# ArthurBrussee/brush

Measured on AMD Instinct MI355X. Metric: train views/sec @ 1M Gaussians, 1080p (fwd + L1/SSIM loss + bwd + Adam per view), higher is better.
Workload: dtype f32

## Files before the change

brush_amd/_ffi.py:

```python
import ctypes as C
import os

_DIR = os.path.dirname(os.path.abspath(__file__))
LIB_PATH = os.environ.get("BRUSH_HIP_LIB") or os.path.join(_DIR, "libbrush_hip.so")

FLAG_MIP = 1
FLAG_BWD_INFO = 2
FLAG_SMOOTH_CUTOFF = 4
FLAG_SLICED_LISTS = 8

fp = C.POINTER(C.c_float)
u32p = C.POINTER(C.c_uint32)


class BhCamera(C.Structure):
    _fields_ = [
        ("vm", C.c_float * 12),
        ("fx", C.c_float), ("fy", C.c_float), ("cx", C.c_float), ("cy", C.c_float),
        ("lim_pos_x", C.c_float), ("lim_pos_y", C.c_float),
        ("lim_neg_x", C.c_float), ("lim_neg_y", C.c_float),
        ("cam_pos", C.c_float * 3),
        ("img_w", C.c_uint32), ("img_h", C.c_uint32),
        ("tile_row_begin", C.c_uint32), ("tile_row_end", C.c_uint32),
        ("model", C.c_uint32), ("dist", C.c_float * 8), ("half_max_render_fov", C.c_float),
# ... 372 lines not shown
    "bh_train_set_features": (C.c_int, [C.c_void_p, C.POINTER(BhFeatureField), C.POINTER(BhFeatureTarget)]),
    "bh_refine_carry_rows": (C.c_int, [C.c_void_p, C.c_void_p, C.c_void_p, C.c_uint32, C.c_uint32]),
}

REGION_BOX, REGION_ELLIPSOID = 0, 1


class BhSceneTransform(C.Structure):
    _fields_ = [("q", C.c_double * 4), ("t", C.c_double * 3), ("s", C.c_double), ("rot", C.c_float * 9), ("quat", C.c_float * 4),
                ("trans", C.c_float * 3), ("scale", C.c_float), ("log_scale", C.c_float), ("sh_rot", C.c_float * 164),
                ("reserved", C.c_uint32 * 2)]


class BhSceneRegion(C.Structure):
    _fields_ = [("kind", C.c_uint32), ("invert", C.c_uint32), ("center", C.c_float * 3), ("half_extent", C.c_float * 3),
                ("rot", C.c_float * 9), ("min_raw_opacity", C.c_float), ("reserved", C.c_uint32)]


SCENE_SYMBOLS = {
    "bh_scene_transform_make": (C.c_int, [dp, dp, C.c_double, C.POINTER(BhSceneTransform)]),
    "bh_scene_transform_compose": (C.c_int, [C.POINTER(BhSceneTransform), C.POINTER(BhSceneTransform), C.POINTER(BhSceneTransform)]),
    "bh_scene_transform_invert": (C.c_int, [C.POINTER(BhSceneTransform), C.POINTER(BhSceneTransform)]),
    "bh_camera_apply_scene_transform": (C.c_int, [C.POINTER(BhCamera), C.POINTER(BhSceneTransform), C.POINTER(BhCamera)]),
    "bh_splats_transform": (C.c_int, [C.c_void_p, C.POINTER(BhSceneTransform), C.c_uint32, C.c_uint32] + [C.c_void_p] * 6),
    "bh_splats_select_region": (C.c_int, [C.c_void_p, C.POINTER(BhSceneRegion), C.c_void_p, C.c_void_p, C.c_uint32, C.c_void_p, u32p]),
}

LIFT_MAX_LABELS, LIFT_UNASSIGNED, LIFT_ANY_LABEL = 256, 255, 0xFFFFFFFF
LIFT_VOTE_ONE = 16777216.0


class BhLiftSelect(C.Structure):
    _fields_ = [("label", C.c_uint32), ("min_share", C.c_float), ("min_weight", C.c_float), ("min_max_weight", C.c_float),
                ("min_pixels", C.c_uint32), ("invert", C.c_uint32)]


LIFT_SYMBOLS = {
    "bh_lift_accumulate": (C.c_int, [C.c_void_p, C.POINTER(BhRenderOut), C.c_void_p, C.c_uint32, C.c_void_p, C.c_void_p, C.c_void_p]),
    "bh_lift_assign": (C.c_int, [C.c_void_p, C.c_void_p, C.c_uint32, C.c_uint32, C.c_float, C.c_void_p, C.c_void_p]),
    "bh_lift_select": (C.c_int, [C.c_void_p, C.c_void_p, C.c_void_p, C.c_void_p, C.c_uint32, C.c_uint32, C.POINTER(BhLiftSelect), C.c_void_p]),
}

ENVMAP_MAX_RESOLUTION = 1024
ENVMAP_SYMBOLS = {
    "bh_envmap_create": (C.c_int, [C.c_void_p, C.c_uint32, C.POINTER(C.c_void_p)]),
    "bh_envmap_destroy": (C.c_int, [C.c_void_p, C.c_void_p]),
    "bh_envmap_set_params": (C.c_int, [C.c_void_p, C.c_void_p, fp]),
    "bh_envmap_get_params": (C.c_int, [C.c_void_p, C.c_void_p, fp]),
    "bh_envmap_get_grad": (C.c_int, [C.c_void_p, C.c_void_p, fp]),
    "bh_envmap_get_state": (C.c_int, [C.c_void_p, C.c_void_p, fp, fp, u32p]),
    "bh_envmap_set_state": (C.c_int, [C.c_void_p, C.c_void_p, fp, fp, C.c_uint32]),
    "bh_envmap_set_adam": (C.c_int, [C.c_void_p, C.c_void_p, C.c_double, C.c_double, C.c_double, C.c_double]),
    "bh_envmap_composite": (C.c_int, [C.c_void_p, C.c_void_p, C.POINTER(BhCamera), C.c_void_p, C.c_uint32, C.c_uint32, C.c_void_p]),
    "bh_envmap_backward": (C.c_int, [C.c_void_p, C.c_void_p, C.POINTER(BhCamera), C.c_void_p, C.c_void_p, C.c_uint32, C.c_uint32, C.c_void_p, C.c_int]),
    "bh_train_set_envmap": (C.c_int, [C.c_void_p, C.c_void_p]),
}

class BhCameraGradTerms(C.Structure):
    _fields_ = [("v_depth", C.c_void_p), ("v_normal", C.c_void_p), ("v_distortion", C.c_void_p), ("depth_mode", C.c_uint32),
                ("normal_mode", C.c_uint32), ("distortion", BhDistortionConfig)]


INTRINSICS_SYMBOLS = {
    "bh_render_backward_intrinsics_saved": (C.c_int, [C.c_void_p, C.POINTER(BhRenderOut)] + [C.c_void_p] * 10),
    "bh_render_backward_camera_saved": (C.c_int, [C.c_void_p, C.POINTER(BhRenderOut), C.c_void_p, C.POINTER(BhCameraGradTerms)] + [C.c_void_p] * 9),
    "bh_train_set_intrinsics_grad": (C.c_int, [C.c_void_p, C.c_void_p]),
    "bh_camera_set_intrinsics": (C.c_int, [C.POINTER(BhCamera), C.c_double, C.c_double, C.c_double, C.c_double]),
}

ABI_VERSION = 7
STRUCT_MIRRORS = (BhCamera, BhRenderOut, BhLossConfig, BhTrainConfig, BhTrainState, BhTrainBatch, BhTrainStats, BhRefineConfig, BhRefineStats, BhPlyInfo)

_lib = None
_lib_th = None
TEST_HOOKS_LIB_PATH = os.path.join(_DIR, "libbrush_hip_testhooks.so")
TEST_HOOK_SYMBOLS = {"bh_debug_fill_train_scratch": (C.c_int, [C.c_void_p, C.c_uint32]),
                     "bh_debug_split_counts": (C.c_int, [C.c_void_p, C.POINTER(C.c_uint32)]),
                     "bh_debug_depth_sort": (C.c_int, [C.c_void_p, C.c_void_p, C.c_void_p, C.c_void_p, C.c_uint32, C.c_void_p, C.c_void_p, C.c_void_p, C.c_void_p,
                                                       C.POINTER(C.c_int), C.POINTER(C.c_uint32)]),
                     "bh_debug_depth_deal": (C.c_int, [C.c_void_p, C.c_void_p, C.c_void_p, C.c_void_p, C.c_uint32, C.c_void_p, C.c_void_p, C.c_void_p, C.c_void_p,
                                                       C.c_uint32, C.c_uint32, C.POINTER(C.c_uint64), C.POINTER(C.c_int)]),
                     "bh_debug_dsort_deal_counts": (C.c_int, [C.c_void_p, C.POINTER(C.c_uint32)]),
                     "bh_debug_set_deal_capacity": (C.c_int, [C.c_void_p, C.c_uint32]),
                     "bh_debug_image_loss_window": (C.c_int, [C.c_void_p, C.c_void_p, C.c_void_p, C.c_uint32, C.c_uint32, C.POINTER(BhLossConfig), C.c_float, C.c_uint32,
                                                              C.c_uint32, C.c_void_p, C.c_void_p])}


class BrushHipError(RuntimeError):
    pass


def _bind(path, symbols):
    if not os.path.exists(path):
        raise BrushHipError(
            "%s not found: build it with `python -c 'import __graft_entry__ as g; g.build()'` "
            "(hipcc --offload-arch=gfx950). There is no CPU fallback." % path)
    lib = C.CDLL(path)
    for name, (res, args) in symbols.items():
        fn = getattr(lib, name)
        fn.restype = res
        fn.argtypes = args
    if lib.bh_abi_version() != ABI_VERSION:
        raise BrushHipError("%s speaks ABI %d, this binding ABI %d" % (path, lib.bh_abi_version(), ABI_VERSION))
    for i, mirror in enumerate(STRUCT_MIRRORS):
        if lib.bh_struct_size(i) != C.sizeof(mirror):
            raise BrushHipError("%s: sizeof(%s) is %d in the library, %d in this binding" % (path, mirror.__name__, lib.bh_struct_size(i), C.sizeof(mirror)))
    return lib


def load():
    global _lib
    if _lib is None:
        _lib = _bind(LIB_PATH, dict(SYMBOLS, **LPIPS_SYMBOLS, **COMPRESSED_PLY_SYMBOLS, **IMAGE_SYMBOLS, **DEPTH_SYMBOLS, **POSE_SYMBOLS, **EXPOSURE_SYMBOLS, **BILAGRID_SYMBOLS, **DEPTH_LOSS_SYMBOLS, **NORMAL_SYMBOLS, **NORMAL_LOSS_SYMBOLS, **DISTORTION_SYMBOLS, **MESH_SYMBOLS, **SPARSE_MESH_SYMBOLS, **FEATURE_SYMBOLS, **FEATURE_TRAIN_SYMBOLS, **SCENE_SYMBOLS, **LIFT_SYMBOLS, **ENVMAP_SYMBOLS, **INTRINSICS_SYMBOLS))
    return _lib


def load_test_hooks():
    global _lib_th
    if _lib_th is None:
        _lib_th = _bind(TEST_HOOKS_LIB_PATH, dict(SYMBOLS, **LPIPS_SYMBOLS, **COMPRESSED_PLY_SYMBOLS, **IMAGE_SYMBOLS, **DEPTH_SYMBOLS, **POSE_SYMBOLS, **EXPOSURE_SYMBOLS, **BILAGRID_SYMBOLS, **DEPTH_LOSS_SYMBOLS, **NORMAL_SYMBOLS, **NORMAL_LOSS_SYMBOLS, **DISTORTION_SYMBOLS, **MESH_SYMBOLS, **SPARSE_MESH_SYMBOLS, **FEATURE_SYMBOLS, **FEATURE_TRAIN_SYMBOLS, **SCENE_SYMBOLS, **LIFT_SYMBOLS, **ENVMAP_SYMBOLS, **INTRINSICS_SYMBOLS,
                                                   **TEST_HOOK_SYMBOLS))
    return _lib_th
```

brush_amd/csrc/api.hip:

```cpp
#include <cmath>
#include <cstdlib>
#include <cstdio>
#include <algorithm>
#include <cstring>
#include <new>

#include "../../include/brush_hip_intrinsics.h"
#include "context.h"
#include "depth_deal.h"
#include "device_rng.h"
#include "param_table.h"

namespace bh {

__global__ __launch_bounds__(256) void zero_two_kernel(float4* __restrict__ a, size_t na, float4* __restrict__ b, size_t nb) {
    const size_t stride = (size_t)gridDim.x * 256;
    const float4 z = make_float4(0.0f, 0.0f, 0.0f, 0.0f);
    for (size_t i = (size_t)blockIdx.x * 256 + threadIdx.x; i < na + nb; i += stride) {
        if (i < na) a[i] = z;
        else b[i - na] = z;
    }
}

int set_error(bh_ctx* ctx, int code, const std::string& msg) {
// ... 166 lines not shown

uint32_t bh_struct_size(uint32_t which) {
    switch (which) {
        case BH_STRUCT_CAMERA: return (uint32_t)sizeof(BhCamera);
        case BH_STRUCT_RENDER_OUT: return (uint32_t)sizeof(BhRenderOut);
        case BH_STRUCT_LOSS_CONFIG: return (uint32_t)sizeof(BhLossConfig);
        case BH_STRUCT_TRAIN_CONFIG: return (uint32_t)sizeof(BhTrainConfig);
        case BH_STRUCT_TRAIN_STATE: return (uint32_t)sizeof(BhTrainState);
        case BH_STRUCT_TRAIN_BATCH: return (uint32_t)sizeof(BhTrainBatch);
        case BH_STRUCT_TRAIN_STATS: return (uint32_t)sizeof(BhTrainStats);
        case BH_STRUCT_REFINE_CONFIG: return (uint32_t)sizeof(BhRefineConfig);
        case BH_STRUCT_REFINE_STATS: return (uint32_t)sizeof(BhRefineStats);
        case BH_STRUCT_PLY_INFO: return (uint32_t)sizeof(BhPlyInfo);
        default: return 0u;
    }
}

bh_ctx* bh_create(int device, void* stream, int own_stream) {
    bh_ctx* ctx = new (std::nothrow) bh_ctx();
    if (!ctx) return nullptr;
    ctx->device = device;
    if (hipSetDevice(device) != hipSuccess) {
        (void)hipGetLastError();
        delete ctx;
        return nullptr;
    }
    if (!own_stream) {
        ctx->stream = (hipStream_t)stream;
        ctx->owns_stream = false;
    } else {
        if (hipStreamCreateWithFlags(&ctx->stream, hipStreamNonBlocking) != hipSuccess) {
            (void)hipGetLastError();
            delete ctx;
            return nullptr;
        }
        ctx->owns_stream = true;
    }
    if (hipHostMalloc((void**)&ctx->host_counters, bh::HOST_COUNTERS_BYTES, hipHostMallocCoherent)    != hipSuccess) {
        (void)hipGetLastError();
        if (ctx->owns_stream) (void)hipStreamDestroy(ctx->stream);
        delete ctx;
        return nullptr;
    }
    std::memset(ctx->host_counters, 0, bh::HOST_COUNTERS_BYTES);
#ifdef BH_TEST_HOOKS
    ctx->knob_break_allreduce = getenv("BH_BREAK_ALLREDUCE") != nullptr;
    if (ctx->knob_break_allreduce)
        fprintf(stderr, "brush_hip: BH_BREAK_ALLREDUCE is set - every all-reduce of this context's communicator is deliberately CORRUPTED (test hook)\n");
    if (const char* e = getenv("BH_TEST_FAIL_LOSS_AT")) {
        ctx->knob_fail_loss_at = (uint32_t)atoi(e);
        if (ctx->knob_fail_loss_at) fprintf(stderr, "brush_hip: BH_TEST_FAIL_LOSS_AT=%u - that train step of this context will FAIL on purpose (test hook)\n", ctx->knob_fail_loss_at);
    }
#endif
    if (hipEventCreateWithFlags(&ctx->readback_ev, hipEventDisableTiming) != hipSuccess ||
        hipEventCreateWithFlags(&ctx->gate_ev, hipEventDisableTiming) != hipSuccess) {
        if (ctx->readback_ev) (void)hipEventDestroy(ctx->readback_ev);
        (void)hipGetLastError();
        (void)hipHostFree(ctx->host_counters);
        if (ctx->owns_stream) (void)hipStreamDestroy(ctx->stream);
        delete ctx;
        return nullptr;
    }
    return ctx;
}

void bh_destroy(bh_ctx* ctx) {
    if (!ctx) return;
    (void)hipSetDevice(ctx->device);
    (void)hipStreamSynchronize(ctx->stream);
    prof_resolve(ctx);
    for (hipEvent_t e : ctx->prof.pool) (void)hipEventDestroy(e);
    for (auto& b : ctx->slots)
        if (b.ptr) (void)hipFree(b.ptr);
    for (auto& kv : ctx->views)
        if (kv.second.zcut) (void)hipFree(kv.second.zcut);
    for (auto& rt : ctx->retained)
        for (auto& b : rt.blocks)
            if (b.ptr) (void)hipFree(b.ptr);
    for (auto& b : ctx->pool)
        if (b.ptr) (void)hipFree(b.ptr);
    if (ctx->host_counters) (void)hipHostFree(ctx->host_counters);
    if (ctx->dsort_spl) (void)hipFree(ctx->dsort_spl);
    if (ctx->deal_ctr) (void)hipFree(ctx->deal_ctr);
    if (ctx->sort_groups) (void)hipFree(ctx->sort_groups);
    if (ctx->readback_ev) (void)hipEventDestroy(ctx->readback_ev);
    if (ctx->gate_ev) (void)hipEventDestroy(ctx->gate_ev);
    if (ctx->image_tab_host) (void)hipHostFree(ctx->image_tab_host);
    if (ctx->image_tab_ev) (void)hipEventDestroy(ctx->image_tab_ev);
    bh::param_tables_free_all(ctx);
    if (ctx->comm) (void)bh_comm_destroy(ctx);
    if (ctx->owns_stream) (void)hipStreamDestroy(ctx->stream);
    delete ctx;
}

const char* bh_last_error(bh_ctx* ctx) { return ctx ? ctx->last_error.c_str() : "null context"; }

int bh_sync(bh_ctx* ctx) {
    if (!ctx) return BH_ERR_INVALID_ARG;
    if (ctx->far_job.pending) {
        BH_HIP(ctx, hipSetDevice(ctx->device));
        BH_TRY(finish_far_slice(ctx, nullptr));
    }
    BH_HIP(ctx, hipStreamSynchronize(ctx->stream));
    deliver_pending_loss(ctx);
    return 0;
}

int bh_profile_enable(bh_ctx* ctx, int on) {
    if (!ctx) return BH_ERR_INVALID_ARG;
    ctx->prof.level = on < 0 ? 0 : (on > 2 ? 1 : on);
    return 0;
}

int bh_profile_fetch(bh_ctx* ctx, const char** names, float* ms, uint32_t* calls, int cap) {
    if (!ctx) return BH_ERR_INVALID_ARG;
    prof_resolve(ctx);
    Profiler& p = ctx->prof;
    const int n = p.count < cap ? p.count : cap;
    for (int i = 0; i < n; ++i) {
        names[i] = p.names[i];
        ms[i] = p.ms[i];
        calls[i] = p.calls[i];
    }
    p.count = 0;
    return n;
}

namespace {
bool parse_u32(const char* v, uint32_t lo, uint32_t hi, uint32_t* out) {
    if (!v || !*v) return false;
    char* end = nullptr;
    const unsigned long long x = strtoull(v, &end, 10);
    if (*end != '\0' || x < lo || x > hi) return false;
    *out = (uint32_t)x;
    return true;
}
bool parse_flag(const char* v, bool* out) {
    uint32_t x = 0;
    if (!parse_u32(v, 0, 1, &x)) return false;
    *out = x != 0;
    return true;
}
struct Option { const char* name; const char* help; bool (*apply)(bh_ctx* c, const char* v); };
const Option kOptions[] = {
    {"cut_min_pairs", "u32: a view whose last frame had fewer pairs keeps complete lists (= bh_set_list_cut_threshold)",
     [](bh_ctx* c, const char* v) { return parse_u32(v, 0, 0xFFFFFFFFu, &c->cut_min_pairs); }},
    {"cut_margin_pct", "0..10000: base margin behind a tile's last useful splat, % of its depth rank (default 150)",
     [](bh_ctx* c, const char* v) { return parse_u32(v, 0, 10000, &c->knob_cut_margin_pct); }},
    {"cut_margin_fixed", "0|1: the margin is cut_margin_pct for every frame instead of adaptive",
     [](bh_ctx* c, const char* v) { return parse_flag(v, &c->knob_fixed_margin); }},
    {"cut_ctrl", "up:down:floor:gap_exp — the margin controller's constants (default 1.5:0.998:0.5:0.3333)", [](bh_ctx* c, const char* v) {
        float a = 0, b = 0, d = 0, e = 0;
        if (sscanf(v, "%f:%f:%f:%f", &a, &b, &d, &e) != 4 || !(a >= 1.0f && b > 0.0f && b <= 1.0f && d > 0.0f && e >= 0.0f && e <= 1.0f)) return false;
        c->ctrl_up = a; c->ctrl_down = b; c->ctrl_floor = d; c->ctrl_gap_exp = e;
        return true;
    }},
    {"cut_sort_all", "0|1: with per-tile cuts, still depth-sort every visible splat",
     [](bh_ctx* c, const char* v) { return parse_flag(v, &c->knob_cut_sort_all); }},
    {"auto_exact_share", "0..1: a view whose last cut frame listed more than this share of its pairs renders complete lists (default 0.9; 0 = never)", [](bh_ctx* c, const char* v) {
        char* end = nullptr;
        const float x = strtof(v, &end);
        if (end == v || *end != '\0' || !(x >= 0.0f && x <= 1.0f)) return false;
        c->auto_exact_share = x;
        return true;
    }},
    {"no_view_hash", "0|1: frames without a view id share ONE table instead of being keyed by their camera",
     [](bh_ctx* c, const char* v) { return parse_flag(v, &c->knob_no_view_hash); }},
    {"k16_order", "0 index order | 1 by the view's last per-tile work | 2 dealt: the forward blend's tile order",
     [](bh_ctx* c, const char* v) { return parse_u32(v, 0, 2, &c->knob_k16_order); }},
    {"band_mode", "0|1: XCD bands of the blend kernels — contiguous eighths of the tile range, or dealt in chunks of 8 adjacent tiles (default 1)",
     [](bh_ctx* c, const char* v) { return parse_u32(v, 0, 1, &c->knob_band_mode); }},
    {"k16_waves", "0..8: forward blend: resident one-wave tiles per SIMD (0 = 8 = all resident at once; fewer: the lighter tiles are dispatched as the heavier ones finish)",
     [](bh_ctx* c, const char* v) { return parse_u32(v, 0, 8, &c->knob_k16_waves); }},
    {"k16_split", "0..1000: forward blend: a tile whose forecast work is at least max(256, k16_split / 100 x its band's mean) is blended by four quadrant waves (default 250; 0: no tile is split)",
     [](bh_ctx* c, const char* v) { return parse_u32(v, 0, 1000, &c->knob_k16_split); }},
    {"k16_split_of_max", "0..100: ... and at least this many percent of its band's heaviest tile (default 45)",
     [](bh_ctx* c, const char* v) { return parse_u32(v, 0, 100, &c->knob_k16_split_of_max); }},
    {"k16_split_min", "1..1023: a tile below this many blended splats (forecast) is never split (default 256)",
     [](bh_ctx* c, const char* v) { return parse_u32(v, 1, 1023, &c->knob_k16_split_min); }},
    {"k5_exact_spw", "16|32|64: splats per wave of the list builder for complete lists",
     [](bh_ctx* c, const char* v) { uint32_t u = 0; if (!parse_u32(v, 16, 64, &u) || !(u == 16 || u == 32 || u == 64)) return false; c->knob_k5_exact_spw = u; return true; }},
    {"bwd_jobs", "0|1: the blend backward works on checkpointed 128-entry segments of the tiles' lists (default 1) or on whole tiles",
     [](bh_ctx* c, const char* v) { return parse_flag(v, &c->knob_bwd_jobs); }},
    {"bwd_wide_rows", "0|1: the blend backward addresses the gradient accumulator in 64 bits, as it does by itself from 2^32 bytes of accumulator on (default 0)",
     [](bh_ctx* c, const char* v) { return parse_flag(v, &c->knob_bwd_wide_rows); }},
    {"no_lpt", "0|1: the blend backward takes its tiles in index order",
     [](bh_ctx* c, const char* v) { return parse_flag(v, &c->knob_no_lpt); }},
    {"lpt_classes", "log|linear: work classes of the backward's longest-first tile order — two per octave of blended splats, or 1/64 of the mean list length wide",
     [](bh_ctx* c, const char* v) { const std::string w(v); if (w == "log") { c->knob_lpt_linear = false; return true; } if (w == "linear") { c->knob_lpt_linear = true; return true; } return false; }},
    {"generic_depth_sort", "0|1: depth order by the generic radix sort + scan instead of the fused split sort",
     [](bh_ctx* c, const char* v) { return parse_flag(v, &c->knob_generic_depth_sort); }},
    {"dsort_splitters", "0|1: the fused depth sort splits at the 254 depth quantiles of the view's previous frame (default 1) or always linearly over the frame's key range",
     [](bh_ctx* c, const char* v) { return parse_flag(v, &c->knob_dsort_splitters); }},
    {"dsort_deal", "0|1: K1 deals the listed splats straight into the depth sort's buckets when the view's splitter table holds quantiles (default 1) or the histogram and split launches always run",
     [](bh_ctx* c, const char* v) { return parse_flag(v, &c->knob_dsort_deal); }},
    {"tile_sort", "auto|bucket|lsd: the forward's tile sort (auto: bucket sort unless the view's pairs are concentrated in few tiles)",
     [](bh_ctx* c, const char* v) { const std::string w(v); if (w == "auto") { c->knob_tile_sort = 0; return true; } if (w == "bucket") { c->knob_tile_sort = 1; return true; } if (w == "lsd") { c->knob_tile_sort = 2; return true; } return false; }},
    {"spec_k5", "0|1: queue the list builder before the host has read the frame's counts (default 1; 0: behind the count readback)",
     [](bh_ctx* c, const char* v) { return parse_flag(v, &c->knob_spec_k5); }},
    {"event_waits", "0|1: the host's mid-step waits use events behind the kernels instead of polled tag words",
     [](bh_ctx* c, const char* v) { return parse_flag(v, &c->knob_event_waits); }},
    {"readback_copy", "0|1: counts and gate word reach the host through copy launches",
     [](bh_ctx* c, const char* v) { return parse_flag(v, &c->knob_readback_copy); }},
    {"force_exchange", "0|1: a one-rank communicator still walks the whole gradient-exchange path (overhead measurement)",
     [](bh_ctx* c, const char* v) { return parse_flag(v, &c->knob_force_exchange); }},
    {"zero_grads", "0|1: the single-GPU train step zero-fills its gradient span like the exchange path",
     [](bh_ctx* c, const char* v) { return parse_flag(v, &c->knob_zero_grads); }},
    {"loss_bands", "0|1: the fused loss's blocks take their tiles by XCD column bands (1) or row-major (0)",
     [](bh_ctx* c, const char* v) { return parse_u32(v, 0, 1, &c->knob_loss_bands); }},
    {"update_rows", "0|64|128|256: splats per block of the update kernel (0 = default)",
     [](bh_ctx* c, const char* v) { uint32_t u = 0; if (!parse_u32(v, 0, 256, &u) || !(u == 0 || u == 64 || u == 128 || u == 256)) return false; c->knob_update_rows = u; return true; }},
    {"no_dormant", "0|1: the update kernel fetches and updates dormant splats like everyone else",
     [](bh_ctx* c, const char* v) { return parse_flag(v, &c->knob_no_dormant); }},
    {"sort_kpt", "0|4|8|16: keys per thread of the generic radix sort (0 = default)",
     [](bh_ctx* c, const char* v) { uint32_t u = 0; if (!parse_u32(v, 0, 16, &u) || !(u == 0 || u == 4 || u == 8 || u == 16)) return false; c->knob_sort_kpt = u; return true; }},
    {"grad_allreduce", "ring|direct: the dense gradient block's collective — ncclAllReduce, or reduce-scatter + all-gather over grouped send/recv",
     [](bh_ctx* c, const char* v) { const std::string w(v); if (w == "ring") { c->knob_direct_allreduce = false; return true; } if (w == "direct") { c->knob_direct_allreduce = true; return true; } return false; }},
    {"update_sparse", "0..256: an update block with at most this many non-dormant rows fetches them in one round trip (0: never; 256: every block that may skip dormant rows; default 64 at SH degree 0, else 0)",
     [](bh_ctx* c, const char* v) { uint32_t u = 0; if (!parse_u32(v, 0, 256, &u)) return false; c->knob_update_sparse = (int)u; return true; }},
    {"feature_chunk", "0|4|8|16: channels per pass over the lists of the feature-map blends (0 = chosen per channel count)",
     [](bh_ctx* c, const char* v) { uint32_t u = 0; if (!parse_u32(v, 0, 16, &u) || !(u == 0 || u == 4 || u == 8 || u == 16)) return false; c->feature_chunk = u; return true; }},
};
constexpr int kOptionCount = (int)(sizeof(kOptions) / sizeof(kOptions[0]));
}

extern "C" int bh_option_count(void) { return kOptionCount; }
extern "C" const char* bh_option_name(int i) { return i >= 0 && i < kOptionCount ? kOptions[i].name : nullptr; }
extern "C" const char* bh_option_help(int i) { return i >= 0 && i < kOptionCount ? kOptions[i].help : nullptr; }

extern "C" int bh_set_option(bh_ctx* ctx, const char* key, const char* value) {
    if (!ctx) return BH_ERR_INVALID_ARG;
    if (!key || !value) return set_error(ctx, BH_ERR_INVALID_ARG, "set_option: null key or value");
    const std::string k(key);
    for (const Option& o : kOptions) {
        if (k != o.name) continue;
        if (!o.apply(ctx, value)) return set_error(ctx, BH_ERR_INVALID_ARG, "set_option: bad value '" + std::string(value) + "' for '" + k + "'");
        return 0;
    }
    return set_error(ctx, BH_ERR_INVALID_ARG, "set_option: unknown key '" + k + "' (bh_option_name lists the keys)");
}

namespace {
struct Kb4Law {
    double k[4];
    explicit Kb4Law(const float* d) { for (int i = 0; i < 4; ++i) k[i] = d ? (double)d[i] : 0.0; }
    double value(double th) const {
        const double t2 = th * th, t3 = t2 * th, t5 = t3 * t2, t7 = t5 * t2, t9 = t7 * t2;
        return th + k[0] * t3 + k[1] * t5 + k[2] * t7 + k[3] * t9;
    }
    double slope(double th) const {
        const double t2 = th * th, t4 = t2 * t2, t6 = t4 * t2, t8 = t6 * t2;
        return 1.0 + 3.0 * k[0] * t2 + 5.0 * k[1] * t4 + 7.0 * k[2] * t6 + 9.0 * k[3] * t8;
    }
    double invert(double target) const {
        if (target <= 0.0) return 0.0;
        const double pi = 3.14159265358979323846;
        double th = target < pi - 1e-6 ? target : pi - 1e-6;
        for (int it = 0; it < 50; ++it) {
            const double fp = slope(th);
            if (std::fabs(fp) < 1e-12) break;
            double next = th - (value(th) - target) / fp;
            next = next < 0.0 ? 0.0 : (next > pi ? pi : next);
            const bool done = std::fabs(next - th) < 1e-12;
            th = next;
            if (done) break;
        }
        return th;
    }
};
struct Rt8Law {
    double k[6];
    explicit Rt8Law(const float* d) { for (int i = 0; i < 6; ++i) k[i] = d ? (double)d[i] : 0.0; }
    double radial(double r) const {
        const double r2 = r * r, r4 = r2 * r2, r6 = r4 * r2;
        return (1.0 + k[0] * r2 + k[1] * r4 + k[2] * r6) / (1.0 + k[3] * r2 + k[4] * r4 + k[5] * r6);
    }
    double undistort(double r_d) const {
        double r = r_d;
// ... 136 lines not shown

extern "C" int bh_render_forward(bh_ctx* ctx, const BhCamera* cam, uint32_t n, uint32_t sh_degree, const float* transforms,
                                 const float* sh_coeffs, const float* raw_opacities, const float* background, uint32_t flags,
                                 BhRenderOut* out) {
    if (!ctx) return BH_ERR_INVALID_ARG;
    if (!cam || !out || !background) return set_error(ctx, BH_ERR_INVALID_ARG, "render_forward: null argument");
    ForwardRequest req;
    req.cam = *cam;
    req.n = n; req.sh_degree = sh_degree; req.flags = flags;
    req.transforms = transforms; req.sh_coeffs = sh_coeffs; req.raw_opacities = raw_opacities;
    req.bg[0] = background[0]; req.bg[1] = background[1]; req.bg[2] = background[2];
    req.view_id = ctx->view_id;
    return render_forward(ctx, req, out);
}

int bh::forward_impl(bh_ctx* ctx, const ForwardRequest& req, BhRenderOut* out) {
    const uint32_t n = req.n, sh_degree = req.sh_degree, flags = req.flags;
    const float* transforms = req.transforms;
    const float* sh_coeffs = req.sh_coeffs;
    const float* raw_opacities = req.raw_opacities;
    ctx->have_forward = false;
    ctx->clears.begin_forward();
    const bool mip = flags & BH_FLAG_MIP;
    Frame f;
    f.bwd_info = flags & BH_FLAG_BWD_INFO; f.smooth = flags & BH_FLAG_SMOOTH_CUTOFF;
    f.bg[0] = req.bg[0]; f.bg[1] = req.bg[1]; f.bg[2] = req.bg[2];
    f.u = make_uniforms(req.cam);
    if (f.u.tile_y0 >= f.u.tile_y1 || f.u.tile_y1 > f.u.tile_bh) return set_error(ctx, BH_ERR_INVALID_ARG, "tile_row window must satisfy begin < end <= ceil(img_h / 16)");
    f.num_tiles = f.u.tile_bw * f.u.tile_bh;
    const size_t npad = n ? n : 1;

    constexpr size_t counter_set_bytes = COUNTER_SET_BYTES, counter_set_words = COUNTER_SET_BYTES / 4, counter_read_bytes = COUNTER_READ_BYTES;
    auto* counter_pairs = (uint32_t*)ensure(ctx, SLOT_COUNTERS, 2 * counter_set_bytes + 64);
    uint32_t* dev_sums = counter_pairs ? counter_pairs + 2 * counter_set_words : nullptr;
    uint32_t* counters = counter_pairs ? counter_pairs + counter_set_words * (ctx->counter_phase & 1u) : nullptr;
    auto* depth_keys = (uint32_t*)ensure(ctx, SLOT_DEPTH_KEYS, npad * 4);
    auto* isect_counts = (uint32_t*)ensure(ctx, SLOT_ISECT_COUNTS, npad * 4);
    auto* max_radius = req.max_radius ? req.max_radius : (float*)ensure(ctx, SLOT_MAX_RADIUS, npad * 4);
    f.proj_by_gid = (float*)ensure(ctx, SLOT_PROJECTED_BY_GID, npad * 9 * 4);
    if (!counters || !depth_keys || !isect_counts || !max_radius || !f.proj_by_gid) return BH_ERR_OOM;

    f.gfc = (uint32_t*)ensure(ctx, SLOT_GLOBAL_FROM_COMPACT, npad * 4);
    auto* depths_sorted = (uint32_t*)ensure(ctx, SLOT_DEPTHS_SORTED, npad * 4);
    if (!f.gfc || !depths_sorted) return BH_ERR_OOM;
    const bool bwd_jobs = f.bwd_info && ctx->knob_bwd_jobs && !ctx->knob_no_lpt && !((flags & BH_FLAG_SLICED_LISTS) && ctx->slice_fraction > 0.0f);
    const size_t lpt_words = LPT_HEADER_WORDS + (size_t)8 * LPT_CLASSES * band_slots(f.num_tiles);
    auto* tile_offsets = (uint32_t*)ensure(ctx, SLOT_TILE_OFFSETS, ((size_t)f.num_tiles * 2 + lpt_words) * 4);
    f.visible = (f.bwd_info && req.visible) ? req.visible : (float*)ensure(ctx, SLOT_VISIBLE, (f.bwd_info ? npad : 1) * 4);
    if (!tile_offsets || !f.visible) return BH_ERR_OOM;
    const size_t visible_words = f.bwd_info ? ((req.visible && req.visible_floats) ? req.visible_floats : npad) : 0;
    const bool want_sliced = (flags & BH_FLAG_SLICED_LISTS) != 0;
    const size_t slice_bit_words = ((size_t)f.num_tiles + 31) / 32;
    const size_t slice_group_words = (size_t)n / (256 * FAR_GROUP_BLOCKS) + 2;
    const size_t slice_words = want_sliced ? SLICE_CTRL_WORDS + slice_bit_words + (size_t)f.num_tiles * 2 + slice_group_words : 0;
    uint32_t* slice_tab = nullptr;
    if (want_sliced) {
        slice_tab = (uint32_t*)ensure(ctx, SLOT_SLICE, slice_words * 4);
        if (!slice_tab) return BH_ERR_OOM;
    }
    ViewState* view = nullptr;
    bool cut_active = false;
    const bool auto_cuts = want_sliced && !(ctx->slice_fraction > 0.0f);
    const bool order_only = !want_sliced && ctx->knob_k16_order != 0u && n >= 8u * 256u;
    if (n > 0 && (auto_cuts || order_only)) {
        view = frame_view(ctx, req, f.u.tile_bw, f.u.tile_bh, order_only && !f.bwd_info);
        if (!view && auto_cuts) return set_error(ctx, BH_ERR_OOM, "hipMalloc for the per-view tile table failed");
        if (!view) (void)hipGetLastError();
        cut_active = auto_cuts && view && cut_this_frame(ctx, view, req.allow_cut);
    }
    uint32_t* const vtab = view_table(view);
    uint32_t* near_counts = nullptr;
    uint32_t* tile_order = nullptr;
    uint32_t* tile_split = nullptr;
    if (cut_active) {
        near_counts = (uint32_t*)ensure(ctx, SLOT_NEAR_COUNTS, npad * 4);
        if (!near_counts) return BH_ERR_OOM;
    }

    uint32_t near_total = 0, nv_true = 0;
    bool fused_scan = false;
    uint32_t* cum_early = nullptr;
    bool k5_queued = false;
    uint32_t spec_pair_cap = 0;
    float* spec_projected = nullptr;
    float4* spec_vc = nullptr;
    uint32_t *spec_tile_ids = nullptr, *spec_isect_gids = nullptr;
    if (n > 0) {
        fused_scan = depth_sort_supported(n) && !ctx->knob_generic_depth_sort;
        const bool sums_on_device = fused_scan && !ctx->knob_readback_copy;
        bool* spl_written = nullptr;
        uint32_t* spl_listed = nullptr;
        uint32_t* spl = view_splitters(view, cut_active, &spl_written, &spl_listed);
        if (!spl && ctx->dsort_spl) { spl = ctx->dsort_spl; spl_written = &ctx->dsort_spl_written; spl_listed = &ctx->dsort_spl_keys; }
        DealArgs dealt;
        {
            ProfScope ps(ctx, "ProjectSplats");
            if (!ctx->counters_ready) BH_HIP(ctx, hipMemsetAsync(counter_pairs, 0, 2 * counter_set_bytes, ctx->stream));
            ctx->counters_ready = false;
            ForwardPrep prep;
            prep.next_counters = reinterpret_cast<unsigned long long*>(counter_pairs + counter_set_words * ((ctx->counter_phase & 1u) ^ 1u));
            prep.visible = visible_words ? reinterpret_cast<uint32_t*>(f.visible) : nullptr;
            prep.visible_words = (uint32_t)visible_words;
            prep.tile_table = tile_offsets;
            prep.tile_words = f.num_tiles * 2 + LPT_HEADER_WORDS;
            prep.slice_table = slice_tab;
            prep.slice_words = (uint32_t)slice_words;
            prep.list_all_visible = ctx->knob_cut_sort_all;
            if (view && ctx->knob_k16_order && n >= 8u * 256u) {
                const uint32_t win_t = f.u.tile_bw * (f.u.tile_y1 - f.u.tile_y0);
                tile_order = (uint32_t*)ensure(ctx, SLOT_TILE_ORDER, ((size_t)8 * band_slots(win_t) + SPLIT_TAIL_WORDS) * 4);
                if (!tile_order) return BH_ERR_OOM;
                prep.order_work = vtab + (size_t)f.num_tiles;
                prep.order_out = tile_order;
                prep.order_tiles = win_t;
                prep.order_tile_begin = f.u.tile_bw * f.u.tile_y0;
                prep.order_mode = ctx->knob_k16_order;
                prep.band_mode = ctx->knob_band_mode;
                if (ctx->knob_k16_split && ctx->knob_k16_order == 1u) {
                    tile_split = tile_order + (size_t)8 * band_slots(win_t);
                    prep.split_out = tile_split;
                    prep.split_factor = (float)ctx->knob_k16_split * 0.01f;
                    prep.split_min = ctx->knob_k16_split_min;
                    prep.split_of_max = (float)ctx->knob_k16_split_of_max * 0.01f;
                }
            }
            if (f.bwd_info && req.grad_begin && req.grad_floats && (req.grad_floats & 3u) == 0 &&
                (reinterpret_cast<uintptr_t>(req.grad_begin) & 15u) == 0 && req.grad_floats / 4 <= 0xFFFFFFFFull) {
                prep.span = reinterpret_cast<float4*>(req.grad_begin);
                prep.span_f4 = (uint32_t)(req.grad_floats / 4);
                ctx->clears.k1_cleared_span();
            }
            BH_TRY(depth_deal_prepare(ctx, n, spl, sums_on_device && spl_written && *spl_written && depth_deal_table_usable(*spl_listed), &prep));
            dealt = prep.deal;
            BH_TRY(launch_project_forward(ctx, f.u, n, mip, sh_degree, transforms, sh_coeffs, raw_opacities, depth_keys, isect_counts, max_radius,
                                          f.proj_by_gid, counters, prep, cut_active ? vtab : nullptr, near_counts));
            ctx->counter_phase ^= 1u;
            ctx->counters_ready = true;
        }
        auto* hslots = reinterpret_cast<unsigned long long*>(ctx->host_counters + 16);
        const bool poll_tag = sums_on_device && !ctx->knob_event_waits;
        if (!sums_on_device) {
            BH_HIP(ctx, hipMemcpyAsync(hslots, counters, counter_read_bytes, hipMemcpyDeviceToHost, ctx->stream));
            BH_HIP(ctx, hipEventRecord(ctx->readback_ev, ctx->stream));
        }
        {
            ProfScope ps(ctx, "DepthSort");
            if (fused_scan) {
                cum_early = (uint32_t*)ensure(ctx, SLOT_CUM_TILES_HIT, npad * 4);
                if (!cum_early) return BH_ERR_OOM;
                if (poll_tag && ++ctx->readback_tag == 0u) ctx->readback_tag = 1u;
                BH_TRY(depth_sort_scan(ctx, depth_keys, counters + COUNTER_MINMAX_WORD, cut_active ? near_counts : isect_counts, n, depths_sorted, f.gfc, cum_early,
                                       sums_on_device ? counters : nullptr, ctx->host_counters + 16, ctx->readback_ev, poll_tag ? ctx->readback_tag : 0u,
                                       sums_on_device ? dev_sums : nullptr, spl, spl_written, &dealt));
            } else {
                BH_TRY(radix_argsort(ctx, depth_keys, nullptr, n, 32, depths_sorted, f.gfc));
            }
        }
        if (poll_tag && ctx->knob_spec_k5 && !(want_sliced && ctx->slice_fraction > 0.0f)) {
            const size_t cap_pairs = std::min(ctx->slots[SLOT_TILE_IDS].cap, ctx->slots[SLOT_ISECT_GIDS].cap) / 4;
            if (cap_pairs >= 4096) {
                spec_projected = (float*)ensure(ctx, SLOT_PROJECTED, npad * 9 * 4);
                spec_vc = f.bwd_info ? (float4*)ensure(ctx, SLOT_V_COMBINED, npad * 10 * 4 + 16) : nullptr;
                if (!spec_projected || (f.bwd_info && !spec_vc)) return BH_ERR_OOM;
                spec_tile_ids = (uint32_t*)ctx->slots[SLOT_TILE_IDS].ptr;
                spec_isect_gids = (uint32_t*)ctx->slots[SLOT_ISECT_GIDS].ptr;
                spec_pair_cap = (uint32_t)std::min<size_t>(cap_pairs, 0xFFFFFFFEull);
                ProfScope ps(ctx, "MapGaussiansToIntersect");
                BH_TRY(launch_map_gaussians(ctx, n, f.u, f.proj_by_gid, f.gfc, spec_projected, cum_early, spec_tile_ids, spec_isect_gids, spec_vc,
                                            spec_vc ? (uint32_t)(((size_t)n * 10 + 3) / 4) : 0u, 0xFFFFFFFFu, cut_active ? slice_tab : nullptr,
                                            cut_active ? vtab : nullptr, cut_active ? depths_sorted : nullptr, dev_sums + (cut_active ? 3 : 0), spec_pair_cap));
                k5_queued = true;
            }
        }
        if (poll_tag) BH_TRY(wait_host_tag(ctx, reinterpret_cast<const volatile uint32_t*>(hslots) + HOST_SUM_WORDS - 1u, ctx->readback_tag, "count readback"));
        else BH_HIP(ctx, hipEventSynchronize(ctx->readback_ev));
        if (ctx->gate_learn) {
            ctx->gate_learn = false;
            ctx->far_direct = reinterpret_cast<const volatile uint32_t*>(ctx->host_counters)[HOST_GATE_WORD] != 0u;
        }
        unsigned long long hc[4] = {0ull, 0ull, 0ull, 0ull};
        if (sums_on_device) {
            const volatile unsigned long long* hs = hslots;
            for (uint32_t c = 0; c < COUNTER_K1_U64; ++c) hc[c] = hs[c];
        } else {
            for (uint32_t k = 0; k < COUNTER_SLOTS; ++k)
                for (uint32_t c = 0; c < COUNTER_K1_U64; ++c) hc[c] += hslots[COUNTER_K1_U64 * k + c];
        }
        if (hc[1] > 0xFFFFFFFFull) return set_error(ctx, BH_ERR_UNSUPPORTED, "more than 2^32-1 tile intersections");
        nv_true = (uint32_t)hc[0];
        f.ni = (uint32_t)hc[1];
        near_total = cut_active ? (uint32_t)hc[2] : f.ni;
        f.nv = cut_active ? (uint32_t)hc[3] : nv_true;
        if (dealt.ctr && reinterpret_cast<const volatile uint32_t*>(hslots)[HOST_DEAL_WORD] != 0u) {
            ProfScope ps(ctx, "DepthSort");
            ctx->deal_fallbacks++;
            BH_TRY(depth_sort_scan(ctx, depth_keys, counters + COUNTER_MINMAX_WORD, cut_active ? near_counts : isect_counts, n, depths_sorted, f.gfc, cum_early,
                                   counters, ctx->host_counters + 16, ctx->readback_ev, 0u, dev_sums, spl, spl_written));
            k5_queued = false;
        }
        if (fused_scan && spl_listed && (spl_written == nullptr || *spl_written)) *spl_listed = f.nv;
    } else {
        BH_HIP(ctx, hipMemsetAsync(tile_offsets, 0, ((size_t)f.num_tiles * 2 + LPT_HEADER_WORDS) * 4, ctx->stream));
        if (visible_words) BH_HIP(ctx, hipMemsetAsync(f.visible, 0, visible_words * 4, ctx->stream));
    }

    const size_t nvpad = f.nv ? f.nv : 1, nipad = f.ni ? f.ni : 1;
    f.cum = fused_scan ? cum_early : (uint32_t*)ensure(ctx, SLOT_CUM_TILES_HIT, nvpad * 4);
    f.projected = (float*)ensure(ctx, SLOT_PROJECTED, nvpad * 9 * 4);
    f.tile_ids = (uint32_t*)ensure(ctx, SLOT_TILE_IDS, nipad * 4);
    f.isect_gids = (uint32_t*)ensure(ctx, SLOT_ISECT_GIDS, nipad * 4);
    f.tile_ids_sorted = (uint32_t*)ensure(ctx, SLOT_TILE_IDS_SORTED, nipad * 4);
    f.isect_gids_sorted = (uint32_t*)ensure(ctx, SLOT_ISECT_GIDS_SORTED, nipad * 4);
    const size_t pixels = (size_t)f.u.img_w * f.u.img_h;
    void* out_img = ensure(ctx, SLOT_OUT_IMG, pixels * (f.bwd_info ? 16 : 4));
    if (!f.cum || !f.projected || !f.tile_ids || !f.isect_gids || !f.tile_ids_sorted || !f.isect_gids_sorted || !out_img)
        return BH_ERR_OOM;
    if (k5_queued && ((cut_active ? near_total : f.ni) > spec_pair_cap || f.projected != spec_projected || f.tile_ids != spec_tile_ids || f.isect_gids != spec_isect_gids))
        k5_queued = false;

    f.budget = want_sliced && f.ni > 0 ? list_budget(ctx, cut_active ? view : nullptr, near_total, f.ni) : f.ni;
    const bool sliced = f.budget < f.ni;
    const bool by_cut = cut_active && sliced;
    const uint32_t* zcut_lists = cut_active ? vtab : nullptr;
    f.slice_info = slice_tab;
    f.done_bits = slice_tab ? slice_tab + SLICE_CTRL_WORDS : nullptr;
    f.tile_offsets_far = slice_tab ? slice_tab + SLICE_CTRL_WORDS + slice_bit_words : nullptr;
    f.far_group_totals = slice_tab ? slice_tab + SLICE_CTRL_WORDS + slice_bit_words + (size_t)f.num_tiles * 2 : nullptr;
    while (f.tile_bits < 32 && (f.num_tiles >> f.tile_bits) != 0) f.tile_bits++;
    if (bwd_jobs) {
        const uint32_t listed = cut_active ? near_total : f.ni;
        const uint32_t ckpt_cap = (uint32_t)std::min<uint64_t>((uint64_t)listed / BWD_SEG + f.num_tiles + 1u, BWD_CKPT_MAX_SLOTS);
        f.rs.jobs.ckpt = (float4*)ensure(ctx, SLOT_BWD_CKPT, (size_t)ckpt_cap * 256 * sizeof(float4));
        f.rs.jobs.ckpt_cap = ckpt_cap;
        f.rs.jobs.top_cap = band_slots(f.num_tiles) + ckpt_cap;
        f.rs.jobs.top_list = (uint32_t*)ensure(ctx, SLOT_BWD_TOPLIST, (size_t)8 * f.rs.jobs.top_cap * 4);
        if (!f.rs.jobs.ckpt || !f.rs.jobs.top_list) return BH_ERR_OOM;
    }
    if (view) {
        f.rs.zcut = vtab;
        f.rs.depth_keys_sorted = depths_sorted;
        f.rs.nv = f.nv;
        f.rs.cut_active = by_cut;
        f.rs.margin_pct = cut_margin_pct(ctx, view);
        f.rs.work = vtab + (size_t)f.num_tiles;
        f.rs.order = tile_order;
        f.rs.order_mode = ctx->knob_k16_order;
        f.rs.split = tile_split;
#ifdef BH_TEST_HOOKS
        ctx->last_split = tile_split;
#endif
    }
    const uint32_t win_tiles = f.u.tile_bw * (f.u.tile_y1 - f.u.tile_y0);
    const float class_width_raw = (float)f.ni / (float)(win_tiles ? win_tiles : 1u) / 64.0f;
    f.class_width = ctx->knob_lpt_linear ? (class_width_raw < 8.0f ? 8.0f : class_width_raw) : 0.0f;
    f.lpt = (f.bwd_info && !ctx->knob_no_lpt) ? tile_offsets + (size_t)f.num_tiles * 2 : nullptr;
    f.out_f32 = f.bwd_info ? (float*)out_img : nullptr;
    f.out_u8 = f.bwd_info ? nullptr : (uint32_t*)out_img;

    bool offsets_done = false;
    if (f.nv > 0) {
        if (!fused_scan) {
            ProfScope ps(ctx, "PrefixSumGaussHits");
            BH_TRY(prefix_sum(ctx, cut_active ? near_counts : isect_counts, f.gfc, f.nv, f.cum, false));
        }
        if (f.ni == 0) {
            ProfScope ps(ctx, "ProjectVisible");
            BH_TRY(launch_project_visible(ctx, f.nv, f.proj_by_gid, f.gfc, f.projected));
        }
        if (f.ni > 0) {
            {
                ProfScope ps(ctx, "MapGaussiansToIntersect");
                float4* vc = nullptr;
                if (f.bwd_info) {
                    vc = (float4*)ensure(ctx, SLOT_V_COMBINED, (size_t)f.nv * 10 * 4 + 16);
                    if (!vc) return BH_ERR_OOM;
                }
                if (zcut_lists && near_total == 0u) {
                } else if (k5_queued && (!f.bwd_info || vc == spec_vc)) {
                    ctx->clears.k5_cleared_accum(vc != nullptr);
                } else {
                    ctx->clears.k5_cleared_accum(vc != nullptr);
                    BH_TRY(launch_map_gaussians(ctx, f.nv, f.u, f.proj_by_gid, f.gfc, f.projected, f.cum, f.tile_ids, f.isect_gids, vc, vc ? (uint32_t)(((size_t)f.nv * 10 + 3) / 4) : 0u,
                                                (sliced && !by_cut) ? f.budget : 0xFFFFFFFFu, (sliced || zcut_lists) ? f.slice_info : nullptr, zcut_lists,
                                                zcut_lists ? depths_sorted : nullptr));
                }
            }
            {
                ProfScope ps(ctx, "TileSort");
                if ((zcut_lists || !sliced) && tile_sort_supported(f.tile_bits, zcut_lists ? near_total : f.ni) && !(ctx->knob_tile_sort == 2u)) {
                    BH_TRY(tile_sort_offsets(ctx, f.tile_ids, f.isect_gids, zcut_lists ? near_total : f.ni, f.tile_bits, f.num_tiles, f.tile_ids_sorted, f.isect_gids_sorted,
                                             tile_offsets, f.ni));
                    offsets_done = true;
                } else
                if (zcut_lists) BH_TRY(radix_argsort_dev(ctx, f.tile_ids, f.isect_gids, near_total, nullptr, nullptr, nullptr, f.tile_bits, f.tile_ids_sorted, f.isect_gids_sorted, f.ni));
                else if (sliced) BH_TRY(radix_argsort_dev(ctx, f.tile_ids, f.isect_gids, f.budget, f.slice_info + 1, nullptr, nullptr, f.tile_bits, f.tile_ids_sorted, f.isect_gids_sorted, f.ni));
                else BH_TRY(radix_argsort(ctx, f.tile_ids, f.isect_gids, f.ni, f.tile_bits, f.tile_ids_sorted, f.isect_gids_sorted));
            }
        }
    }
    if (!offsets_done) {
        ProfScope ps(ctx, "GetTileOffsets");
        if (zcut_lists) BH_TRY(launch_tile_offsets(ctx, f.tile_ids_sorted, near_total, f.num_tiles, tile_offsets, true));
        else if (sliced) BH_TRY(launch_tile_offsets_dev(ctx, f.tile_ids_sorted, f.budget, f.slice_info + 1, nullptr, nullptr, f.num_tiles, tile_offsets));
        else BH_TRY(launch_tile_offsets(ctx, f.tile_ids_sorted, f.ni, f.num_tiles, tile_offsets, true));
    }
    if (!sliced) {
        ProfScope ps(ctx, "Rasterize");
        BH_TRY(launch_rasterize(ctx, f.u, f.bg, f.bwd_info, f.smooth, f.isect_gids_sorted, tile_offsets, f.projected, f.gfc, f.out_f32, f.out_u8, f.visible, f.lpt,
                                f.class_width, 0, &f.rs));
    } else {
        auto* state = (float*)ensure(ctx, SLOT_SLICE_STATE, pixels * 16);
        f.far_counts = (uint32_t*)ensure(ctx, SLOT_SLICE_COUNTS, nvpad * 4);
        f.far_block_totals = (uint32_t*)ensure(ctx, SLOT_SLICE_CUM, (nvpad / 256 + 2) * 4);
        if (!state || !f.far_counts || !f.far_block_totals) return BH_ERR_OOM;
        f.rs.done_bits = f.done_bits;
        f.rs.unsat_count = f.slice_info + 2;
        if (!ctx->knob_readback_copy) {
            f.rs.gate_host = ctx->host_counters + HOST_GATE_WORD;
            *reinterpret_cast<volatile uint32_t*>(f.rs.gate_host) = 0u;
        }
        f.rs.state = state;
        f.rs.offsets_near = tile_offsets;
        f.rs.live_bands = f.slice_info + 4;
        {
            ProfScope ps(ctx, "Rasterize");
            BH_TRY(launch_rasterize(ctx, f.u, f.bg, f.bwd_info, f.smooth, f.isect_gids_sorted, tile_offsets, f.projected, f.gfc, f.out_f32, f.out_u8, f.visible, f.lpt,
                                    f.class_width, 1, &f.rs));
        }
        FarJob& j = ctx->far_job;
        j.frame = f;
        j.by_cut = by_cut;
        j.view = by_cut ? view : nullptr;
        j.view_shared = req.view_id == 0u && ctx->knob_no_view_hash;
        if (by_cut) j.req = req;
        if (ctx->knob_readback_copy)
            BH_HIP(ctx, hipMemcpyAsync(ctx->host_counters + HOST_GATE_WORD, f.slice_info + 2, 4, hipMemcpyDeviceToHost, ctx->stream));
        if (ctx->far_direct && !by_cut) {
            BH_TRY(enqueue_far_slice(ctx, j));
            ctx->gate_learn = true;
        } else {
            if (++ctx->gate_tag == 0u) ctx->gate_tag = 1u;
            j.gate_tag = ctx->gate_tag;
            ctx->gate_signal_queued = false;
            j.gate_event_recorded = !(req.defer_decision && !ctx->knob_event_waits && !ctx->knob_readback_copy);
            if (j.gate_event_recorded) BH_HIP(ctx, hipEventRecord(ctx->gate_ev, ctx->stream));
            j.pending = true;
            if (!req.defer_decision) {
                bool again = false;
                BH_TRY(finish_far_slice(ctx, &again));
                if (by_cut && again) {
                    *out = ctx->latest.out;
                    return 0;
                }
            }
        }
    }

    BhRenderOut r{};
    r.num_visible = nv_true;
    r.num_listed_splats = f.nv;
    r.num_intersections = f.ni;
    r.num_tiles = f.num_tiles;
    r.tile_bw = f.u.tile_bw;
    r.tile_bh = f.u.tile_bh;
// ... 403 lines not shown
    if (n == 0) return 0;
    if (tile_sort_supported(bits, n) && !(ctx->knob_tile_sort == 2u))
        return tile_sort_offsets(ctx, tile_ids, compact_gids, n, bits, num_tiles, tile_ids_sorted, compact_gids_sorted, tile_offsets);
    BH_TRY(radix_argsort(ctx, tile_ids, compact_gids, n, bits, tile_ids_sorted, compact_gids_sorted));
    return launch_tile_offsets(ctx, tile_ids_sorted, n, num_tiles, tile_offsets, true);
}

#ifdef BH_TEST_HOOKS
extern "C" int bh_debug_split_counts(bh_ctx* ctx, uint32_t* out) {
    if (!ctx || !out) return BH_ERR_INVALID_ARG;
    if (!ctx->last_split) return 0;
    BH_HIP(ctx, hipSetDevice(ctx->device));
    BH_HIP(ctx, hipMemcpyAsync(out, ctx->last_split, 8 * 4, hipMemcpyDeviceToHost, ctx->stream));
    BH_HIP(ctx, hipStreamSynchronize(ctx->stream));
    return 1;
}
extern "C" int bh_debug_depth_sort(bh_ctx* ctx, const uint32_t* keys, const uint32_t* minmax, const uint32_t* counts, uint32_t n, uint32_t* out_keys, uint32_t* out_vals,
                                   uint32_t* cum, uint32_t* spl, int* spl_written, uint32_t* totals_out) {
    if (!ctx) return BH_ERR_INVALID_ARG;
    if (!keys || !minmax || !counts || !out_keys || !out_vals || !cum || !totals_out || (spl && !spl_written))
        return set_error(ctx, BH_ERR_INVALID_ARG, "debug_depth_sort: null argument");
    if (n == 0 || !depth_sort_supported(n)) return set_error(ctx, BH_ERR_INVALID_ARG, "debug_depth_sort: n is outside the fused sort's reach");
    BH_HIP(ctx, hipSetDevice(ctx->device));
    bool written = spl_written ? *spl_written != 0 : false;
    BH_TRY(depth_sort_scan(ctx, keys, minmax, counts, n, out_keys, out_vals, cum, nullptr, nullptr, nullptr, 0u, nullptr, spl, spl ? &written : nullptr));
    if (spl) *spl_written = written ? 1 : 0;
    else if (spl_written) *spl_written = ctx->dsort_spl_written ? 1 : 0;
    BH_HIP(ctx, hipMemcpyAsync(totals_out, ctx->slots[SLOT_SORT_HIST].ptr, 2 * 256 * 4, hipMemcpyDeviceToHost, ctx->stream));
    BH_HIP(ctx, hipStreamSynchronize(ctx->stream));
    return 0;
}
__global__ __launch_bounds__(256) void debug_deal_kernel(const uint32_t* __restrict__ keys, const uint32_t* __restrict__ counts, uint32_t n, uint32_t stride, bh::DealArgs d) {
    __shared__ uint32_t s_spl[bh::DEAL_SPL_WORDS];
    bh::deal_stage(d, s_spl);
    __syncthreads();
    const uint32_t t = blockIdx.x * 256u + threadIdx.x;
    if (t >= n) return;
    const uint32_t e = (uint32_t)(((unsigned long long)t * stride) % n);
    const uint32_t key = keys[e];
    if (key != 0xFFFFFFFFu) bh::deal_put(d, bh::deal_take(d, s_spl, key, counts[e]), key, e);
}
extern "C" int bh_debug_depth_deal(bh_ctx* ctx, const uint32_t* keys, const uint32_t* minmax, const uint32_t* counts, uint32_t n, uint32_t* out_keys, uint32_t* out_vals,
                                   uint32_t* cum, uint32_t* spl, uint32_t cap, uint32_t stride, unsigned long long* ctr_out, int* fell_back) {
    if (!ctx) return BH_ERR_INVALID_ARG;
    if (!keys || !minmax || !counts || !out_keys || !out_vals || !cum || !spl || !ctr_out || !fell_back || stride == 0u)
        return set_error(ctx, BH_ERR_INVALID_ARG, "debug_depth_deal: bad argument");
    if (n == 0 || !depth_sort_supported(n)) return set_error(ctx, BH_ERR_INVALID_ARG, "debug_depth_deal: n is outside the fused sort's reach");
    BH_HIP(ctx, hipSetDevice(ctx->device));
    DealArgs d;
    d.spl = spl;
    d.cap = cap ? cap : deal_capacity(n);
    d.region = (uint2*)ensure(ctx, SLOT_DEAL_REGION, (size_t)DEAL_BUCKETS * d.cap * sizeof(uint2));
    if (!d.region) return BH_ERR_OOM;
    if (hipMalloc((void**)&d.ctr, (size_t)DEAL_SET_U64 * 8) != hipSuccess) { (void)hipGetLastError(); return BH_ERR_OOM; }
    int rc = check_hip(ctx, hipMemsetAsync(d.ctr, 0, (size_t)DEAL_SET_U64 * 8, ctx->stream), "debug_depth_deal: clear");
    if (rc == 0) {
        hipLaunchKernelGGL(debug_deal_kernel, dim3((n + 255u) / 256u), dim3(256), 0, ctx->stream, keys, counts, n, stride, d);
        rc = check_hip(ctx, hipGetLastError(), "debug_deal_kernel");
    }
    bool written = true;
    if (rc == 0) rc = depth_sort_scan(ctx, keys, minmax, counts, n, out_keys, out_vals, cum, nullptr, nullptr, nullptr, 0u, nullptr, spl, &written, &d);
    unsigned long long host[DEAL_BUCKETS + 1u];
    if (rc == 0) rc = check_hip(ctx, hipMemcpy2DAsync(host, 8, d.ctr, (size_t)DEAL_LINE_U64 * 8, 8, DEAL_BUCKETS + 1u, hipMemcpyDeviceToHost, ctx->stream), "debug_depth_deal: counters");
    if (rc == 0) rc = check_hip(ctx, hipStreamSynchronize(ctx->stream), "debug_depth_deal: sync");
    if (rc == 0) {
        for (uint32_t i = 0; i <= DEAL_BUCKETS; ++i) ctr_out[i] = host[i];
        *fell_back = host[DEAL_BUCKETS] != 0ull ? 1 : 0;
        if (*fell_back) {
            ctx->deal_fallbacks++;
            rc = depth_sort_scan(ctx, keys, minmax, counts, n, out_keys, out_vals, cum, nullptr, nullptr, nullptr, 0u, nullptr, spl, &written);
            if (rc == 0) rc = check_hip(ctx, hipStreamSynchronize(ctx->stream), "debug_depth_deal: sync");
        }
    } else {
        (void)hipStreamSynchronize(ctx->stream);
    }
    (void)hipFree(d.ctr);
    return rc;
}
extern "C" int bh_debug_set_deal_capacity(bh_ctx* ctx, uint32_t cap) {
    if (!ctx) return BH_ERR_INVALID_ARG;
    ctx->deal_cap_override = cap;
    return 0;
}
extern "C" int bh_debug_dsort_deal_counts(bh_ctx* ctx, uint32_t* out) {
    if (!ctx || !out) return BH_ERR_INVALID_ARG;
    out[0] = ctx->deal_frames;
    out[1] = ctx->deal_fallbacks;
    return 0;
}
extern "C" int bh_debug_image_loss_window(bh_ctx* ctx, const float* img_hwc4, const uint32_t* gt_packed, uint32_t h, uint32_t w, const BhLossConfig* cfg,
                                          float alpha_weight, uint32_t tile_y0, uint32_t tile_y1, float* loss_out, float* v_output) {
    if (!ctx) return BH_ERR_INVALID_ARG;
    if (!img_hwc4 || !gt_packed || !cfg || !loss_out || !v_output || h == 0 || w == 0)
        return set_error(ctx, BH_ERR_INVALID_ARG, "debug_image_loss_window: bad argument");
    if (tile_y0 >= tile_y1) return set_error(ctx, BH_ERR_INVALID_ARG, "debug_image_loss_window: empty tile-row window");
    BH_HIP(ctx, hipSetDevice(ctx->device));
    const size_t hw = (size_t)h * w;
    const bool alpha = alpha_weight > 0.0f;
    BH_TRY(launch_image_loss_fused_window(ctx, img_hwc4, gt_packed, h, w, *cfg, alpha, 1.0f / (float)(hw * 3), alpha ? alpha_weight / (float)hw : 0.0f, tile_y0,
                                          tile_y1, loss_out, v_output, nullptr, nullptr, 0u));
    BH_HIP(ctx, hipStreamSynchronize(ctx->stream));
    return 0;
}
#endif
```

brush_amd/csrc/context.h:

```cpp
#pragma once
#include <hip/hip_runtime.h>
#include <stdint.h>

#include <memory>
#include <string>
#include <unordered_map>
#include <vector>

#include "../../include/brush_hip.h"
#include "../../include/brush_hip_lpips.h"
#include "../../include/brush_hip_image.h"
#include "../../include/brush_hip_exposure.h"
#include "../../include/brush_hip_bilagrid.h"
#include "../../include/brush_hip_depth_loss.h"
#include "../../include/brush_hip_normal_loss.h"
#include "../../include/brush_hip_distortion.h"
#include "../../include/brush_hip_mesh.h"
#include "../../include/brush_hip_features.h"
#include "../../include/brush_hip_feature_train.h"
#include "../../include/brush_hip_envmap.h"
#include "device_math.h"

namespace bh {

enum Slot : int {
    SLOT_COUNTERS = 0,
    SLOT_DEPTH_KEYS,
    SLOT_ISECT_COUNTS,
    SLOT_MAX_RADIUS,
    SLOT_SORT_KEYS_A,
    SLOT_SORT_KEYS_B,
    SLOT_SORT_VALS_A,
    SLOT_SORT_VALS_B,
    SLOT_SORT_HIST,
    SLOT_COMM_SCRATCH,
    SLOT_BWD_CKPT,
    SLOT_BWD_TOPLIST,
    SLOT_SORT_PARTS,
    SLOT_SCAN_SUMS,
    SLOT_GLOBAL_FROM_COMPACT,
    SLOT_DEPTHS_SORTED,
    SLOT_CUM_TILES_HIT,
    SLOT_PROJECTED,
    SLOT_TILE_IDS,
    SLOT_ISECT_GIDS,
    SLOT_TILE_IDS_SORTED,
    SLOT_ISECT_GIDS_SORTED,
    SLOT_TILE_OFFSETS,
    SLOT_OUT_IMG,
    SLOT_VISIBLE,
    SLOT_V_COMBINED,
    SLOT_LOSS_MAP,
    SLOT_V_OUTPUT,
    SLOT_GRADS,
    SLOT_STATS,
    SLOT_LOSS_SCALAR,
    SLOT_MISC,
    SLOT_REFINE,
    SLOT_REFINE_BOUNDS,
    SLOT_FOLDED_TRANSFORMS,
    SLOT_FOLDED_RAW_OPAC,
    SLOT_PLY_ROWS,
    SLOT_EXCH_BLOCKS,
    SLOT_EXCH_IDX,
    SLOT_EXCH_COMPACT,
    SLOT_PROJECTED_BY_GID,
    SLOT_SLICE,
    SLOT_SLICE_STATE,
    SLOT_SLICE_COUNTS,
    SLOT_SLICE_CUM,
    SLOT_NEAR_COUNTS,
    SLOT_TILE_ORDER,
    SLOT_LOD_GRADS,
    SLOT_LOD_FOLDED,
    SLOT_LOD_LOSS,
    SLOT_LOD_SORT,
    SLOT_KNN,
    SLOT_EVAL,
    SLOT_LPIPS,
    SLOT_PLY_COMPRESS,
    SLOT_IMAGE,
    SLOT_DEPTH,
    SLOT_POSE,
    SLOT_INTRINSICS,
    SLOT_EXPOSURE,
    SLOT_CORRECTED,
    SLOT_PIXEL_LOSS,
    SLOT_DEPTH_TERM,
    SLOT_NORMAL,
    SLOT_NORMAL_TERM,
    SLOT_DISTORTION,
    SLOT_DISTORTION_TERM,
    SLOT_BILAGRID,
    SLOT_TSDF,
    SLOT_FEATURES,
    SLOT_FEATURE_TERM,
    SLOT_FEATURE_GRAD,
    SLOT_ENVMAP_FRAME,
    SLOT_DEAL_REGION,
    SLOT_SCENE,
    SLOT_SPTSDF,
    SLOT_COUNT
};

struct Buffer {
    void* ptr = nullptr;
    size_t cap = 0;
};

constexpr int MAX_PROF = 32;

constexpr uint32_t COUNTER_SLOTS = 128;
constexpr uint32_t COUNTER_K1_U64 = 4;
constexpr size_t COUNTER_SET_BYTES = COUNTER_SLOTS * 8 * COUNTER_K1_U64 + COUNTER_SLOTS * 8;
constexpr uint32_t COUNTER_SET_U64 = (uint32_t)(COUNTER_SET_BYTES / 8);
constexpr uint32_t COUNTER_MINMAX_WORD = COUNTER_SLOTS * 2 * COUNTER_K1_U64;
constexpr uint32_t SLICE_CTRL_WORDS = 8;
constexpr uint32_t SORT_GROUP_BLOCKS = 32;
constexpr uint32_t FAR_GROUP_BLOCKS = 64;
constexpr size_t COUNTER_READ_BYTES = COUNTER_SLOTS * 8 * COUNTER_K1_U64;
constexpr uint32_t HOST_SUM_WORDS = 2 * COUNTER_K1_U64 + 1;
constexpr uint32_t HOST_DEAL_WORD = HOST_SUM_WORDS;
constexpr size_t HOST_LOSS_WORD = 16 + COUNTER_READ_BYTES / 4;
constexpr size_t HOST_GATE_WORD = HOST_LOSS_WORD + 16;
constexpr size_t HOST_GATE_TAG_WORD = HOST_GATE_WORD + 1;
constexpr size_t HOST_COUNTERS_BYTES = 64 + COUNTER_READ_BYTES + 64 + 64;

struct Profiler {
    int level = 0;
    const char* names[MAX_PROF];
    float ms[MAX_PROF];
    uint32_t calls[MAX_PROF];
    int count = 0;
    struct Pending { int idx; hipEvent_t a, b; };
    std::vector<Pending> pending;
    std::vector<hipEvent_t> pool;
    hipEvent_t ext_a = nullptr, ext_b = nullptr;
};

constexpr uint32_t ZCUT_ALL = 0xFFFFFFFEu;
BH_DEV bool zcut_near(uint32_t key, uint32_t cut) { return (key >> 1) <= (cut >> 1); }
struct ViewState {
    uint32_t* zcut = nullptr;
    uint32_t tile_bw = 0, tile_bh = 0;
    bool seeded = false;
    uint32_t exact_frames = 0;
    uint32_t penalty = 0;
    uint64_t last_used = 0;
    uint32_t gap = 0;
    uint32_t last_pairs = 0;
    uint32_t complete_frames = 0;
    bool spl_written[2] = {false, false};
    uint32_t spl_keys[2] = {0, 0};
    bool casual = false;
};
constexpr uint32_t CUT_MIN_PAIRS = 1500000u;
constexpr uint32_t LPT_CLASSES = 64;
constexpr uint32_t LPT_HEADER_WORDS = 8 * LPT_CLASSES + 64;
constexpr uint32_t BWD_SEG = 128;
constexpr uint32_t BWD_MAX_SEGS = 64;
struct BwdJobs {
    float4* ckpt = nullptr;
    uint32_t ckpt_cap = 0;
    uint32_t* top_list = nullptr;
    uint32_t top_cap = 0;
};
constexpr uint32_t BAND_CHUNK = 4;
inline __host__ __device__ uint32_t band_slots(uint32_t num_tiles) {
    const uint32_t p = (num_tiles + 7u) / 8u;
    return ((p + BAND_CHUNK - 1u) / BAND_CHUNK) * BAND_CHUNK;
}
inline __host__ __device__ uint32_t band_tile(uint32_t band, uint32_t i, uint32_t per, uint32_t mode) {
    return mode ? ((i / BAND_CHUNK) * 8u + band) * BAND_CHUNK + (i % BAND_CHUNK) : band * per + i;
}
BH_DEV uint32_t tile_of_block(uint32_t b, uint32_t num_tiles, uint32_t band_mode) {
    const uint32_t per = band_slots(num_tiles);
    const uint32_t i = b >> 3;
    return i < per ? band_tile(b & 7u, i, per, band_mode) : 0xFFFFFFFFu;
}
constexpr uint32_t SPLIT_MAX = 128;
constexpr uint32_t SPLIT_MIN_WORK = 256;
constexpr uint32_t SPLIT_TAIL_WORDS = 8u + 8u * SPLIT_MAX * 4u;
constexpr uint32_t BWD_CKPT_MAX_SLOTS = 96u * 1024u;
constexpr uint32_t DSORT_SPL_STRIDE = 260;
constexpr uint32_t VIEW_SPL_WORDS = 2 * DSORT_SPL_STRIDE;
constexpr uint32_t DEAL_BUCKETS = 255;
constexpr uint32_t DEAL_LINE_U64 = 16;
constexpr uint32_t DEAL_SET_U64 = (DEAL_BUCKETS + 1u) * DEAL_LINE_U64;
constexpr uint32_t DEAL_OVERFLOW_U64 = DEAL_BUCKETS * DEAL_LINE_U64;
struct DealArgs {
    const uint32_t* spl = nullptr;
    unsigned long long* ctr = nullptr;
    uint2* region = nullptr;
    uint32_t cap = 0;
};
constexpr size_t MAX_VIEW_STATES = 4096;
constexpr uint64_t DIRECT_ALLREDUCE_MIN_FLOATS = 1u << 16;
constexpr uint32_t AUTO_EXACT_FRAMES = 12;
constexpr size_t CASUAL_VIEW_STATES = 32;
constexpr size_t SEEN_KEYS = 64;
constexpr size_t VIEW_TABLE_BYTES = (size_t)256 << 20;

struct RasterSlice {
    uint32_t* done_bits = nullptr;
    uint32_t* unsat_count = nullptr;
    uint32_t* gate_host = nullptr;
    float* state = nullptr;
    const uint32_t* offsets_near = nullptr;
    uint32_t* zcut = nullptr;
    const uint32_t* depth_keys_sorted = nullptr;
    uint32_t nv = 0;
    bool cut_active = false;
    uint32_t* live_bands = nullptr;
    uint32_t* work = nullptr;
    const uint32_t* order = nullptr;
    uint32_t order_mode = 1;
    uint32_t* split = nullptr;
    uint32_t margin_pct = 150;
    BwdJobs jobs{};
};

struct ForwardRequest {
    BhCamera cam{};
    uint32_t n = 0, sh_degree = 0, flags = 0;
    const float* transforms = nullptr;
    const float* sh_coeffs = nullptr;
    const float* raw_opacities = nullptr;
    float bg[3] = {0, 0, 0};
    uint32_t view_id = 0;
    float* visible = nullptr;
    float* max_radius = nullptr;
    size_t visible_floats = 0;
    float* grad_begin = nullptr;
    size_t grad_floats = 0;
    bool defer_decision = false;
    bool allow_cut = true;
};

struct Frame {
    ViewUniforms u{};
    float bg[3] = {0, 0, 0};
    bool bwd_info = false, smooth = false;
    uint32_t nv = 0, ni = 0, budget = 0, num_tiles = 0, tile_bits = 0;
    float* proj_by_gid = nullptr;
    uint32_t* gfc = nullptr;
    float* projected = nullptr;
    uint32_t* cum = nullptr;
    uint32_t* slice_info = nullptr;
    uint32_t* done_bits = nullptr;
    uint32_t* tile_offsets_far = nullptr;
    uint32_t* far_counts = nullptr;
    uint32_t* far_block_totals = nullptr;
    uint32_t* far_group_totals = nullptr;
    uint32_t* tile_ids = nullptr;
    uint32_t* isect_gids = nullptr;
    uint32_t* tile_ids_sorted = nullptr;
    uint32_t* isect_gids_sorted = nullptr;
    float* out_f32 = nullptr;
    uint32_t* out_u8 = nullptr;
    float* visible = nullptr;
    uint32_t* lpt = nullptr;
    float class_width = 8.0f;
    RasterSlice rs{};
};

struct FarJob {
    bool pending = false;
    Frame frame{};
    bool gate_event_recorded = false;
    uint32_t gate_tag = 0;
    bool by_cut = false;
    ViewState* view = nullptr;
    bool view_shared = false;
    ForwardRequest req{};
};

struct GradClears {
// ... 78 lines not shown
    float* pose_grad = nullptr;
    float* intrinsics_grad = nullptr;
    bool depth_attached = false;
    BhDepthTarget depth_target{};
    bool normal_attached = false;
    BhNormalTermConfig normal_term{};
    bool distortion_attached = false;
    BhDistortionTermConfig distortion_term{};
    bool feature_attached = false;
    BhFeatureField feature_field{};
    BhFeatureTarget feature_target{};
    bh_exposure* exposure = nullptr;
    bh_bilagrid* bilagrid = nullptr;
    float bilagrid_tv_weight = 0.0f;
    bh_envmap* envmap = nullptr;

    bool lpips_on() const { return lpips != nullptr && lpips_weight > 0.0f; }
    bool depth_on() const { return depth_attached && depth_target.weight > 0.0f; }
    bool normal_on() const { return normal_attached && normal_term.weight > 0.0f; }
    bool distortion_on() const { return distortion_attached; }
    bool feature_on() const { return feature_attached && feature_target.weight > 0.0f; }
};

}


struct bh_ctx {
    int device = 0;
    hipStream_t stream = nullptr;
    bool owns_stream = false;
    std::string last_error;
    bh::Buffer slots[bh::SLOT_COUNT];
    uint32_t* host_counters = nullptr;
    hipEvent_t readback_ev = nullptr;
    hipEvent_t gate_ev = nullptr;
    bool counters_ready = false;
    uint32_t counter_phase = 0;
    bool have_forward = false;
    bh::ForwardState latest;
    uint64_t generation = 0;
    std::vector<bh::Retained> retained;
    std::vector<bh::Buffer> pool;
    bh::GradClears clears;
    float* pending_loss_dst = nullptr;
    void* image_tab_host = nullptr;
    size_t image_tab_cap = 0;
    hipEvent_t image_tab_ev = nullptr;
    bh::StepTerms terms;
    std::vector<bh::ParamTable*> param_tables;
    void* comm = nullptr;
    hipStream_t comm_stream = nullptr;
    hipEvent_t comm_ev = nullptr;
    int comm_rank = 0, comm_world = 1;
    float slice_fraction = 0.0f;
    float last_slice_share = 1.0f;
    bool far_direct = false;
    uint32_t readback_tag = 0;
    uint32_t gate_tag = 0;
    bool gate_signal_queued = false;
    bool gate_learn = false;
    uint32_t far_launches = 0;
    std::unordered_map<uint64_t, bh::ViewState> views;
    uint64_t seen_keys[bh::SEEN_KEYS] = {};
    uint32_t seen_pos = 0;
    uint32_t casual_views = 0;
    uint32_t view_id = 0;
    uint64_t view_clock = 0;
    float margin_scale = 1.0f;
    float ctrl_up = 1.5f, ctrl_down = 0.998f, ctrl_floor = 0.5f, ctrl_gap_exp = 1.0f / 3.0f;
    uint32_t cut_min_pairs = bh::CUT_MIN_PAIRS;
    bool knob_spec_k5 = true;
    bool knob_event_waits = false;
    bool knob_readback_copy = false;
    bool knob_no_view_hash = false;
    bool knob_fixed_margin = false;
    bool knob_cut_sort_all = false;
    uint32_t feature_chunk = 0;
    uint32_t knob_band_mode = 1;
    uint32_t knob_k16_waves = 0;
    uint32_t knob_k16_split = 250;
    uint32_t knob_k16_split_min = bh::SPLIT_MIN_WORK;
    uint32_t knob_k16_split_of_max = 45;
    const uint32_t* last_split = nullptr;
    uint32_t knob_k16_order = 1;
    uint32_t knob_cut_margin_pct = 150;
    bh::FarJob far_job;
    uint32_t refine_n = 0, refine_new_n = 0;
    bool dsort_deal_lds_raised = false;
    bool dsort_lds_raised = false;
    uint32_t* sort_groups = nullptr;
    size_t sort_groups_cap = 0, sort_groups_dirty = 0;
    uint32_t sort_groups_cur = 0;
    uint32_t* dsort_spl = nullptr;
    bool dsort_spl_written = false;
    uint32_t dsort_spl_keys = 0;
    unsigned long long* deal_ctr = nullptr;
    uint32_t deal_phase = 0;
    uint32_t deal_frames = 0, deal_fallbacks = 0;
    uint32_t deal_cap_override = 0;
    bool knob_dsort_deal = true;
    bool knob_dsort_splitters = true;
    bool adam_lds_raised = false;
    uint32_t update_lds_raised = 0;
    size_t lds_optin_max = 0;
    bool knob_no_lpt = false;
    bool knob_bwd_wide_rows = false;
    bool knob_bwd_jobs = true;
    bool knob_lpt_linear = false;
    bool knob_force_exchange = false;
    bool knob_break_allreduce = false;
    bool knob_generic_depth_sort = false;
    bool knob_zero_grads = false;
    uint32_t knob_fail_loss_at = 0;
    uint32_t train_steps_seen = 0;
    uint32_t knob_loss_bands = 1;
    uint32_t knob_tile_sort = 0;
    float auto_exact_share = 0.9f;
    bool knob_direct_allreduce = false;
    uint32_t knob_k5_exact_spw = 32;
    bool knob_no_dormant = false;
    int knob_update_sparse = -1;
    uint32_t knob_update_rows = 0;
    uint32_t knob_sort_kpt = 0;
    const void* marks_m2_sh = nullptr; const void* marks_m1_t = nullptr; uint32_t marks_n = 0, marks_step = 0;
    bh::Profiler prof;
};

namespace bh {

int set_error(bh_ctx* ctx, int code, const std::string& msg);
int forward_impl(bh_ctx* ctx, const ForwardRequest& req, BhRenderOut* out);
int wait_host_tag(bh_ctx* ctx, const volatile uint32_t* word, uint32_t want, const char* what);
int find_saved_bwd_forward(bh_ctx* ctx, const BhRenderOut* saved, int not_bwd_code, const char* who, const ForwardState** fs);
int backward_impl(bh_ctx* ctx, const ForwardState& fs, const float* v_output, const BackwardCall& call);
int render_forward(bh_ctx* ctx, const ForwardRequest& req, BhRenderOut* out);
enum : uint32_t { NEED_V_OUTPUT = 1u, NEED_V_DEPTH = 2u, NEED_V_NORMAL = 4u, NEED_V_DISTORTION = 8u, NEED_V_VIEWMAT = 16u, NEED_V_FEATURES = 32u, NEED_V_INTRINSICS = 64u };
int backward_entry(bh_ctx* ctx, const char* who, int not_bwd_code, uint32_t required, const BhRenderOut* saved, const float* v_output, BackwardCall call);
int launch_depth_backward(bh_ctx* ctx, const ForwardState& fs, const DepthTerm& term, float* v_combined, float** v_z);
int launch_depth_vz_scatter(bh_ctx* ctx, const ForwardState& fs, const float* v_z, float* v_transforms, bool mark_rows, float* v_sh_coeffs,
                            float* v_raw_opacities, float* v_refine_weight);
int launch_depth_forward(bh_ctx* ctx, const ForwardState& fs, uint32_t mode, float* out_depth);
int launch_normal_backward(bh_ctx* ctx, const ForwardState& fs, const NormalTerm& term, const float* transforms, float* v_combined, const float** v_n);
int launch_normal_vn_scatter(bh_ctx* ctx, const ForwardState& fs, const float* v_n, const float* transforms, float* v_transforms, bool mark_rows,
                             float* v_sh_coeffs, float* v_raw_opacities, float* v_refine_weight);
int launch_normal_map(bh_ctx* ctx, const ForwardState& fs, const float* transforms, uint32_t mode, float* out);
int launch_normal_loss(bh_ctx* ctx, const BhCamera& cam, const float* normal, const float* depth, const float* image, uint32_t h, uint32_t w, float weight,
                       bool accumulate_v_depth, float* loss, float* v_normal, float* v_depth, float* accum, float* accum_host);
int launch_distortion_backward(bh_ctx* ctx, const ForwardState& fs, const DistortionTerm& term, float* v_combined, float** v_z);
int launch_distortion_map(bh_ctx* ctx, const ForwardState& fs, const DistortionTerm& term, bool moments, float* out);
int check_distortion_kind(bh_ctx* ctx, uint32_t kind, float near_z, float far_z, const char* who);
int launch_distortion_loss(bh_ctx* ctx, const float* map, uint32_t h, uint32_t w, uint32_t channels, float weight, float* loss, float* accum,
                           float* accum_host);
int launch_feature_backward(bh_ctx* ctx, const ForwardState& fs, const FeatureTerm& term, float* v_combined, const float** v_compact);
int launch_feature_scatter(bh_ctx* ctx, const ForwardState& fs, const FeatureTerm& term, const float* v_compact);
int launch_feature_gather(bh_ctx* ctx, const ForwardState& fs, const float* features, uint32_t channels, float* feat);
int launch_feature_forward(bh_ctx* ctx, const ForwardState& fs, uint32_t channels, const float* feat, float* out);
int feature_term_rows(bh_ctx* ctx, const ForwardState& fs, uint32_t channels, float** feat);
int launch_feature_loss(bh_ctx* ctx, const float* map, const BhFeatureTarget& t, float* loss, float* v_map, float* accum, float* accum_host);
int launch_depth_loss(bh_ctx* ctx, const float* depth, const BhDepthTarget& t, float* loss, float* v_depth, float* accum, float* accum_host);
double* loss_partials(bh_ctx* ctx, uint64_t pixels, uint32_t* blocks);
int launch_loss_pair_final(bh_ctx* ctx, uint32_t rows, const double* partials, float c, float* loss, float* accum, float* accum_host);
int launch_pose_grad(bh_ctx* ctx, const ViewUniforms& u, uint32_t nv, bool mip, uint32_t sh_degree, const float* transforms,
                     const float* sh, const uint32_t* gid, const float* v_combined, float* v_viewmat);
int launch_intrinsics_grad(bh_ctx* ctx, const ViewUniforms& u, uint32_t nv, bool mip, const float* transforms, const uint32_t* gid,
                           const float* v_combined, float* v_intrinsics);
int launch_exposure_apply(bh_ctx* ctx, const bh_exposure* tab, uint32_t view, const float* img, uint32_t h, uint32_t w, float* out);
int launch_exposure_backward(bh_ctx* ctx, bh_exposure* tab, uint32_t view, const float* img, const float* v_exposed, uint32_t h, uint32_t w,
                             float* v_img, bool update);
int launch_bilagrid_slice(bh_ctx* ctx, const bh_bilagrid* tab, uint32_t view, const float* img, uint32_t h, uint32_t w, float* out);
int launch_bilagrid_backward(bh_ctx* ctx, bh_bilagrid* tab, uint32_t view, const float* img, const float* v_sliced, uint32_t h, uint32_t w, float* v_img,
                             float tv_weight, bool update);
int launch_bilagrid_tv(bh_ctx* ctx, const bh_bilagrid* tab, uint32_t view, float* value, float weight, float* accum, float* accum_host);
float* bilagrid_tv_scratch(bh_ctx* ctx);
int check_envmap_frame(bh_ctx* ctx, const BhCamera* cam, uint32_t h, uint32_t w, const char* who);
int launch_envmap_composite(bh_ctx* ctx, const bh_envmap* map, const BhCamera& cam, const float* img, uint32_t h, uint32_t w, float* out);
int launch_envmap_backward(bh_ctx* ctx, bh_envmap* map, const BhCamera& cam, const float* img, const float* v_out, uint32_t h, uint32_t w, float* v_img,
                           bool update, float gscale, bool check_host);
int launch_envmap_adam(bh_ctx* ctx, bh_envmap* map, float gscale);
ViewState* frame_view(bh_ctx* ctx, const ForwardRequest& req, uint32_t tile_bw, uint32_t tile_bh, bool casual);
bool cut_this_frame(const bh_ctx* ctx, ViewState* vs, bool allow_cut);
uint32_t* view_table(const ViewState* vs);
uint32_t* view_splitters(ViewState* vs, bool cut, bool** written, uint32_t** listed = nullptr);
uint32_t cut_margin_pct(const bh_ctx* ctx, const ViewState* vs);
uint32_t list_budget(bh_ctx* ctx, ViewState* cut_view, uint32_t near_total, uint32_t ni);
void view_rendered(ViewState* vs, uint32_t ni);
int enqueue_far_slice(bh_ctx* ctx, const FarJob& j);
int finish_far_slice(bh_ctx* ctx, bool* launched);
bool far_job_decides_first(const bh_ctx* ctx);
void drop_far_job(bh_ctx* ctx);
inline void deliver_pending_loss(bh_ctx* ctx) {
    if (ctx->pending_loss_dst) {
        *ctx->pending_loss_dst = reinterpret_cast<const volatile float*>(ctx->host_counters)[HOST_LOSS_WORD];
        ctx->pending_loss_dst = nullptr;
    }
}
int check_hip(bh_ctx* ctx, hipError_t e, const char* what);
int lpips_train_term(bh_ctx* ctx, const float* img_hwc4, const uint32_t* gt_packed, uint32_t h, uint32_t w, const float* bg, float* v_output,
                     float* loss, float* loss_host);
std::string ply_header_comments(uint32_t sh_degree, bool render_mip, const float* up_axis);
enum ResizeOut : int { RESIZE_OUT_U8 = 0, RESIZE_OUT_PACKED = 1, RESIZE_OUT_PACKED_PREMUL = 2 };
size_t resize_table_bytes(uint32_t src, uint32_t dst, uint32_t filter);
void build_resize_table(uint32_t src, uint32_t dst, uint32_t filter, void* host);
using ResizeTable = std::shared_ptr<const std::vector<uint8_t>>;
ResizeTable resize_table(uint32_t src, uint32_t dst, uint32_t filter);
hipError_t enqueue_resize(hipStream_t st, const uint8_t* src, uint32_t w, uint32_t h, uint32_t channels, uint32_t nw, uint32_t nh,
                          const int32_t* vtab, const int32_t* htab, float* tmp, void* out, int mode);
hipError_t enqueue_mask_merge(hipStream_t st, const uint8_t* img, uint32_t channels, const uint8_t* mask, uint64_t pixels, int invert,
                              int premultiply, uint32_t* out);
void* ensure(bh_ctx* ctx, Slot s, size_t bytes);

struct ProfScope {
    bh_ctx* ctx;
    int idx = -1;
    hipEvent_t a = nullptr, b = nullptr;
    ProfScope(bh_ctx* c, const char* name, bool dominant = false);
    ~ProfScope();
};

#define BH_HIP(ctx, expr)                                            \
    do {                                                             \
        hipError_t _e = (expr);                                      \
        if (_e != hipSuccess) return bh::check_hip(ctx, _e, #expr);  \
    } while (0)
#define BH_TRY(expr)            \
    do {                        \
        int _rc = (expr);       \
        if (_rc != 0) return _rc; \
    } while (0)
#define BH_LAUNCH_CHECK(ctx, what)                                      \
    do {                                                                \
        hipError_t _e = hipGetLastError();                              \
        if (_e != hipSuccess) return bh::check_hip(ctx, _e, what);      \
    } while (0)

ViewUniforms make_uniforms(const BhCamera& c);


struct ForwardPrep {
    unsigned long long* next_counters = nullptr;
    uint32_t* visible = nullptr;
    uint32_t visible_words = 0;
    uint32_t* tile_table = nullptr;
    uint32_t tile_words = 0;
    float4* span = nullptr;
    uint32_t span_f4 = 0;
    uint32_t* slice_table = nullptr;
    uint32_t slice_words = 0;
    const uint32_t* order_work = nullptr;
    uint32_t* order_out = nullptr;
    uint32_t order_tiles = 0, order_tile_begin = 0;
    uint32_t order_mode = 1;
    uint32_t band_mode = 0;
    uint32_t* split_out = nullptr;
    float split_factor = 2.5f;
    uint32_t split_min = SPLIT_MIN_WORK;
    float split_of_max = 0.45f;
    bool list_all_visible = false;
    DealArgs deal;
    unsigned long long* deal_next = nullptr;
};
int launch_project_forward(bh_ctx* ctx, const ViewUniforms& u, uint32_t n, bool mip, uint32_t sh_degree, const float* transforms,
                           const float* sh, const float* raw_opac, uint32_t* depth_keys, uint32_t* isect_counts, float* max_radius,
                           float* projected_by_gid, uint32_t* counters, const ForwardPrep& prep, uint32_t* zcut = nullptr,
                           uint32_t* near_counts = nullptr);
int launch_project_visible(bh_ctx* ctx, uint32_t nv, const float* projected_by_gid, const uint32_t* gid, float* projected);
int launch_map_gaussians(bh_ctx* ctx, uint32_t nv, const ViewUniforms& u, const float* projected_by_gid, const uint32_t* gid,
                         float* projected, const uint32_t* cum_tiles_hit, uint32_t* tile_ids, uint32_t* isect_gids,
                         float4* zero_span = nullptr, uint32_t zero_f4 = 0, uint32_t budget = 0xFFFFFFFFu, uint32_t* slice_info = nullptr,
                         const uint32_t* zcut = nullptr, const uint32_t* depth_keys_sorted = nullptr, const uint32_t* nv_dev = nullptr, uint32_t pair_cap = 0xFFFFFFFFu);
int launch_map_gaussians_far(bh_ctx* ctx, uint32_t nv, const ViewUniforms& u, const float* projected_by_gid, const uint32_t* gid,
                             float* projected, const uint32_t* cum_tiles_hit, uint32_t budget, const uint32_t* done_bits, const uint32_t* gate,
                             uint32_t* counts, uint32_t* block_totals, uint32_t* group_totals, uint32_t* slice_info, uint32_t* tile_ids, uint32_t* isect_gids);
int launch_project_backward(bh_ctx* ctx, const ViewUniforms& u, uint32_t nv, bool mip, uint32_t sh_degree,
                            const float* transforms, const float* sh, const float* raw_opac, const uint32_t* gid,
                            float* v_combined, float* v_transforms, float* v_sh, float* v_raw_opac,
                            float* v_refine, bool mark_written = false, const float* projected = nullptr);
struct SortGroups {
    uint32_t* sums = nullptr;
    uint32_t* stale = nullptr;
    uint32_t stale_words = 0;
};
inline uint32_t sort_group_count(uint32_t nblocks) { return (nblocks + SORT_GROUP_BLOCKS - 1u) / SORT_GROUP_BLOCKS; }
int sort_groups_next(bh_ctx* ctx, size_t words, SortGroups* out);
constexpr uint32_t SORT_DIRECT_GROUPS = 32;
inline bool sort_groups_scanned(uint32_t ngroups) { return ngroups > SORT_DIRECT_GROUPS; }
int sort_groups_scan(bh_ctx* ctx, uint32_t* sums, uint32_t ngroups, uint32_t tables, uint32_t* totals);
int radix_argsort(bh_ctx* ctx, const uint32_t* keys, const uint32_t* vals, uint32_t n, uint32_t bits,
                  uint32_t* out_keys, uint32_t* out_vals);
int radix_argsort_dev(bh_ctx* ctx, const uint32_t* keys, const uint32_t* vals, uint32_t n_max, const uint32_t* n_dev, const uint32_t* gate,
                      const uint32_t* out_base, uint32_t bits, uint32_t* out_keys, uint32_t* out_vals, uint32_t alloc_n = 0);
bool tile_sort_supported(uint32_t bits, uint32_t n);
int tile_sort_offsets(bh_ctx* ctx, const uint32_t* keys, const uint32_t* vals, uint32_t n, uint32_t bits, uint32_t num_tiles,
                      uint32_t* out_keys, uint32_t* out_vals, uint32_t* tile_offsets, uint32_t alloc_n = 0);
bool depth_sort_supported(uint32_t n);
int depth_sort_scan(bh_ctx* ctx, const uint32_t* keys, const uint32_t* minmax, const uint32_t* counts, uint32_t n, uint32_t* out_keys,
                    uint32_t* out_vals, uint32_t* cum, const uint32_t* rb_set = nullptr, uint32_t* rb_host = nullptr, hipEvent_t rb_done = nullptr,
                    uint32_t rb_tag = 0, uint32_t* rb_dev = nullptr, uint32_t* spl = nullptr, bool* spl_written = nullptr, const DealArgs* dealt = nullptr);
int depth_deal_prepare(bh_ctx* ctx, uint32_t n, const uint32_t* spl, bool table_usable, ForwardPrep* prep);
bool depth_deal_table_usable(uint32_t listed_by_writer);
int prefix_sum(bh_ctx* ctx, const uint32_t* in, const uint32_t* gather, uint32_t n, uint32_t* out, bool exclusive, const uint32_t* gate = nullptr);
int launch_tile_offsets(bh_ctx* ctx, const uint32_t* tile_ids_sorted, uint32_t num_isect, uint32_t num_tiles,
                        uint32_t* tile_offsets, bool pre_zeroed = false);
int launch_tile_offsets_dev(bh_ctx* ctx, const uint32_t* tile_ids_sorted, uint32_t n_max, const uint32_t* n_dev, const uint32_t* gate,
                            const uint32_t* base, uint32_t num_tiles, uint32_t* tile_offsets);

int launch_rasterize(bh_ctx* ctx, const ViewUniforms& u, const float bg[3], bool bwd_info, bool smooth,
                     const uint32_t* isect_gids, uint32_t* tile_offsets, const float* projected,
                     const uint32_t* global_from_compact, float* out_img, uint32_t* out_packed, float* visible,
                     uint32_t* lpt, float class_width, int phase = 0, const RasterSlice* slice = nullptr);
int launch_rasterize_backward(bh_ctx* ctx, const ViewUniforms& u, const float bg[3], bool smooth,
                              const uint32_t* isect_gids, const uint32_t* tile_offsets, const float* projected,
                              const float* out_img, const float* v_output, float* v_combined, const uint32_t* lpt,
                              const uint32_t* tile_offsets_far = nullptr, bool want_refine = true, const BwdJobs* jobs = nullptr,
                              uint32_t accum_rows = 0u);
int launch_image_loss_forward(bh_ctx* ctx, const float* pred, const uint32_t* gt, uint32_t channels, uint32_t h,
                              uint32_t w, const BhLossConfig& cfg, float* loss_map);
int launch_image_loss_backward(bh_ctx* ctx, const float* pred, const uint32_t* gt, const float* dl_dmap,
                               float dl_const, uint32_t channels, uint32_t h, uint32_t w, const BhLossConfig& cfg,
                               float* dl_dpred);
int launch_image_loss_fused(bh_ctx* ctx, const float* img_hwc4, const uint32_t* gt, uint32_t h, uint32_t w, const BhLossConfig& cfg,
                            bool alpha_match, float dl_rgb, float dl_alpha, float* loss_out, float* v_output, float* loss_host = nullptr,
                            uint32_t* started_host = nullptr, uint32_t started_tag = 0);
int launch_image_loss_fused_window(bh_ctx* ctx, const float* img_hwc4, const uint32_t* gt, uint32_t h, uint32_t w, const BhLossConfig& cfg,
                                   bool alpha_match, float dl_rgb, float dl_alpha, uint32_t tile_y0, uint32_t tile_y1, float* loss_out,
                                   float* v_output, float* loss_host = nullptr, uint32_t* started_host = nullptr, uint32_t started_tag = 0);
int launch_adam(bh_ctx* ctx, float* param, const float* grad, float* m1, float* m2, uint64_t rows, uint32_t row_len,
                const float* col_scale, float lr, uint32_t t, bool reduce_m2, float beta1, float beta2, float eps, float gscale = 1.0f);
struct NoiseArgs { uint64_t seed; uint32_t step; float scale, clamp_abs; };
struct UpdateCall {
    const float *g_transforms, *g_sh, *g_opac;
    const float *refine_weight, *visible, *screen_radius;
    float gscale;
    bool vis_clamp;
    float tab_t[10];
    float lr_sh, sh_rest_scale, lr_opac;
    uint32_t t;
    float beta1, beta2, eps;
    const NoiseArgs* noise;
    bool masked_rows;
};
int launch_train_update(bh_ctx* ctx, const BhTrainState* st, const UpdateCall& c);
int launch_gather_stats(bh_ctx* ctx, float* refine_weight_norm, float* vis_weight, float* max_screen_size,
                        const float* refine_weight, const float* visible, const float* screen_radius, uint64_t n);
int launch_mean_noise(bh_ctx* ctx, float* transforms, const float* raw_opac, const float* visible,
                      const float* samples, uint64_t n, float noise_scale, float clamp_abs, uint64_t seed = 0, uint32_t step = 0);
int launch_normal_samples(bh_ctx* ctx, float* out, uint64_t n, uint64_t seed, uint32_t step);

int launch_fold_min_scale(bh_ctx* ctx, const float* transforms, const float* raw_opac, const float* min_scale, uint32_t n,
                          float* out_transforms, float* out_raw_opac);
int launch_fold_min_scale_backward(bh_ctx* ctx, const float* transforms, const float* raw_opac, const float* min_scale, uint32_t n,
                                   float* v_transforms, float* v_raw_opac);
int launch_compute_min_scale(bh_ctx* ctx, const float* transforms, uint32_t n, const float* view_cams, uint32_t k, float factor, float* out);
// ... 11 lines not shown
```

brush_amd/csrc/depth_sort.hip:

```cpp
#include <cstddef>

#include "context.h"
#include "depth_deal.h"
#include "sort_groups.h"

namespace bh {

constexpr int DS_WG = 256;
constexpr int DS_WAVES = DS_WG / 64;
#define BH_DS_KPT 8
constexpr int DS_KPT = BH_DS_KPT;
constexpr int DS_TILE = DS_WG * DS_KPT;
constexpr int DS_RADIX = 256;
constexpr uint32_t CULLED_KEY = 0xFFFFFFFFu;

struct DepthSplit {
    uint32_t kmin, kmax;
    uint32_t scale;
    bool any_visible;
    const uint32_t* spl;
};
constexpr uint32_t SPL_WORDS = 258;
static_assert(SPL_WORDS <= DSORT_SPL_STRIDE, "context.h reserves the table");
constexpr uint32_t SPL_MIN_KEYS = 16384;
// ... 5 lines not shown
    sp.any_visible = nmin != 0u;
    sp.kmin = ~nmin;
    sp.kmax = kmax;
    const uint32_t range = sp.any_visible ? kmax - sp.kmin : 0u;
    sp.scale = (uint32_t)min((unsigned long long)0xFFFFFFFFull, (255ull << 32) / ((unsigned long long)range + 1ull));
    if ((((unsigned long long)range * sp.scale) >> 32) > 254ull) sp.scale -= 1u;
    sp.spl = nullptr;
    return sp;
}

BH_DEV DepthSplit depth_split(const uint32_t* __restrict__ minmax, uint32_t* s_red , const uint32_t* __restrict__ spl_in ,
                              uint32_t* s_spl ) {
    const int tid = threadIdx.x, lane = tid & 63, wave = tid >> 6;
    uint32_t a = 0, b = 0;
    if (tid < (int)COUNTER_SLOTS) {
        a = minmax[2 * tid];
        b = minmax[2 * tid + 1];
    }
    if (spl_in != nullptr) {
        s_spl[tid] = spl_in[tid];
        if (tid < (int)SPL_WORDS - DS_WG) s_spl[DS_WG + tid] = spl_in[DS_WG + tid];
    }
#pragma unroll
    for (int off = 32; off > 0; off >>= 1) {
        a = max(a, (uint32_t)__shfl_xor((int)a, off));
        b = max(b, (uint32_t)__shfl_xor((int)b, off));
    }
    if (lane == 0) { s_red[wave] = a; s_red[DS_WAVES + wave] = b; }
    __syncthreads();
    uint32_t kmax = 0, nmin = 0;
#pragma unroll
    for (int w = 0; w < DS_WAVES; ++w) { kmax = max(kmax, s_red[w]); nmin = max(nmin, s_red[DS_WAVES + w]); }
    __syncthreads();
    DepthSplit sp = make_split(kmax, nmin);
    if (spl_in != nullptr && sp.any_visible && s_spl[255] != 0u) {
        const uint32_t tmin = s_spl[256], tmax = s_spl[257], tol = (tmax - tmin) >> 4;
        const uint32_t dmin = sp.kmin > tmin ? sp.kmin - tmin : tmin - sp.kmin, dmax = sp.kmax > tmax ? sp.kmax - tmax : tmax - sp.kmax;
        if (dmin <= tol && dmax <= tol) sp.spl = s_spl;
    }
    return sp;
}
BH_DEV uint32_t depth_digit(uint32_t key, const DepthSplit& sp) {
    if (key == CULLED_KEY) return 255u;
    if (sp.spl != nullptr) {
        uint32_t d = 0;
#pragma unroll
        for (uint32_t step = 128u; step != 0u; step >>= 1) d += sp.spl[d + step - 1u] <= key ? step : 0u;
        return d;
    }
    return min(254u, (uint32_t)(((unsigned long long)(key - sp.kmin) * sp.scale) >> 32));
}

BH_DEV unsigned long long ds_match(uint32_t d) {
    uint32_t lo = 0xFFFFFFFFu, hi = 0xFFFFFFFFu;
#pragma unroll
    for (int b = 0; b < 8; ++b) {
        const uint32_t bit = (d >> b) & 1u;
        const unsigned long long bal = __ballot(bit);
        const uint32_t flip = bit - 1u;
        lo &= (uint32_t)bal ^ flip;
        hi &= (uint32_t)(bal >> 32) ^ flip;
    }
    return ((unsigned long long)hi << 32) | lo;
}

BH_DEV void counter_sums_to_host(const uint32_t* __restrict__ set, uint32_t* __restrict__ host_sums, int lane, uint32_t tag, uint32_t* __restrict__ dev_sums,
                                 uint32_t deal_overflow = 0u) {
    const unsigned long long* c64 = reinterpret_cast<const unsigned long long*>(set);
    unsigned long long tot[COUNTER_K1_U64];
#pragma unroll
    for (uint32_t c = 0; c < COUNTER_K1_U64; ++c) tot[c] = 0ull;
    for (uint32_t k = (uint32_t)lane; k < COUNTER_SLOTS; k += 64u) {
#pragma unroll
        for (uint32_t c = 0; c < COUNTER_K1_U64; ++c) tot[c] += c64[COUNTER_K1_U64 * k + c];
    }
#pragma unroll
    for (int off = 32; off > 0; off >>= 1) {
#pragma unroll
        for (uint32_t c = 0; c < COUNTER_K1_U64; ++c) tot[c] += __shfl_down(tot[c], off);
    }
    if (lane == 0) {
        if (dev_sums) {
#pragma unroll
            for (uint32_t c = 0; c < COUNTER_K1_U64; ++c) dev_sums[c] = deal_overflow ? 0u : (tot[c] > 0xFFFFFFFFull ? 0xFFFFFFFFu : (uint32_t)tot[c]);
        }
        volatile unsigned long long* h64 = reinterpret_cast<volatile unsigned long long*>(host_sums);
#pragma unroll
        for (uint32_t c = 0; c < COUNTER_K1_U64; ++c) h64[c] = tot[c];
        reinterpret_cast<volatile uint32_t*>(host_sums)[HOST_DEAL_WORD] = deal_overflow;
        if (tag) {
            __threadfence_system();
            reinterpret_cast<volatile uint32_t*>(host_sums)[HOST_SUM_WORDS - 1u] = tag;
        }
    }
}

__global__ __launch_bounds__(DS_WG) void dsort_hist_kernel(const uint32_t* __restrict__ keys, const uint32_t* __restrict__ counts,
                                                          uint32_t n, uint32_t nblocks, const uint32_t* __restrict__ minmax,
                                                          uint32_t* __restrict__ hist , SortGroups grp, uint32_t ngroups,
                                                          const uint32_t* __restrict__ rb_set, uint32_t* __restrict__ rb_host, uint32_t rb_tag, uint32_t* __restrict__ rb_dev,
                                                          const uint32_t* __restrict__ spl_in, uint8_t* __restrict__ digits ) {
    __shared__ uint32_t s_hist[DS_WAVES][DS_RADIX];
    __shared__ uint32_t s_csum[DS_WAVES][DS_RADIX];
    __shared__ uint32_t s_red[2 * DS_WAVES];
    __shared__ uint32_t s_spl[SPL_WORDS];
    const int tid = threadIdx.x, wave = tid >> 6;
    sort_groups_clear(grp.stale, grp.stale_words);
    if (blockIdx.x == nblocks) {
        if (wave == 0) counter_sums_to_host(rb_set, rb_host, tid, rb_tag, rb_dev);
        return;
    }
    for (int i = tid; i < DS_WAVES * DS_RADIX; i += DS_WG) { (&s_hist[0][0])[i] = 0; (&s_csum[0][0])[i] = 0; }
    const DepthSplit sp = depth_split(minmax, s_red, spl_in, s_spl);
    const uint32_t base = blockIdx.x * DS_TILE;
    auto count_one = [&](uint32_t key, uint32_t cnt) {
        const uint32_t d = depth_digit(key, sp);
        if (d != 255u) {
            atomicAdd(&s_hist[wave][d], 1u);
            atomicAdd(&s_csum[wave][d], cnt);
        }
        return d;
    };
    if (base + (uint32_t)DS_TILE <= n && ((reinterpret_cast<uintptr_t>(keys) | reinterpret_cast<uintptr_t>(counts)) & 15u) == 0) {
        const uint4* k4 = reinterpret_cast<const uint4*>(keys + base);
        const uint4* c4 = reinterpret_cast<const uint4*>(counts + base);
        uint4 kv[DS_KPT / 4], cv[DS_KPT / 4];
#pragma unroll
        for (int k = 0; k < DS_KPT / 4; ++k) { kv[k] = k4[k * DS_WG + tid]; cv[k] = c4[k * DS_WG + tid]; }
        uint32_t* d4 = reinterpret_cast<uint32_t*>(digits + base);
#pragma unroll
        for (int k = 0; k < DS_KPT / 4; ++k) {
            const uint32_t d0 = count_one(kv[k].x, cv[k].x);
            const uint32_t d1 = count_one(kv[k].y, cv[k].y);
            const uint32_t d2 = count_one(kv[k].z, cv[k].z);
            const uint32_t d3 = count_one(kv[k].w, cv[k].w);
            d4[k * DS_WG + tid] = d0 | (d1 << 8) | (d2 << 16) | (d3 << 24);
        }
    } else {
#pragma unroll
        for (int k = 0; k < DS_KPT; ++k) {
            const uint32_t idx = base + k * DS_WG + tid;
            if (idx < n) digits[idx] = (uint8_t)count_one(keys[idx], counts[idx]);
        }
    }
    __syncthreads();
    uint32_t t = 0, c = 0;
#pragma unroll
    for (int w = 0; w < DS_WAVES; ++w) { t += s_hist[w][tid]; c += s_csum[w][tid]; }
    hist[(size_t)blockIdx.x * DS_RADIX + tid] = t;
    const size_t gw = (size_t)(blockIdx.x / SORT_GROUP_BLOCKS) * DS_RADIX + tid;
    if (t != 0u) atomicAdd(&grp.sums[gw], t);
    if (c != 0u) atomicAdd(&grp.sums[(size_t)ngroups * DS_RADIX + gw], c);
}

template <int WG>
struct ChunkLds {
    uint32_t cnt[WG / 64][DS_RADIX];
    uint32_t dbase[DS_RADIX];
    uint32_t gofs[DS_RADIX];
    uint32_t wsum[WG / 64];
    uint32_t keys[DS_TILE];
    uint32_t vals[DS_TILE];
    uint8_t digs[DS_TILE];
};
template <int WG, class DigitFn>
BH_DEV void scatter_chunk(ChunkLds<WG>& L, uint32_t* __restrict__ s_base , const uint32_t* __restrict__ src_k,
                          const uint32_t* __restrict__ src_v , uint32_t first, uint32_t count, uint32_t* __restrict__ dst_k,
// ... 648 lines not shown
```

brush_amd/csrc/project.hip:

```cpp
#include "context.h"
#include "depth_deal.h"
#include "device_camera.h"
#include "device_f64_sum.h"
#include "device_sh.h"

namespace bh {

constexpr int PROJ_WG = 256;
constexpr int PROJ_WAVES = PROJ_WG / 64;
constexpr uint32_t ORDER_BINS = 1024;

struct WalkLds {
    uint32_t count[64];
    float mx[64], my[64], c00[64], c01[64], c11[64], pt[64];
    uint32_t magic[64];
    uint32_t box[64];
    uint32_t boxw[64];
    uint32_t start[64];
    uint32_t lane_of[64];
    uint32_t zkey[64];
    uint32_t near[64];
    uint8_t flags[64];
};

BH_DEV uint32_t walk_magic(uint32_t bw, uint32_t nb) {
    if (bw < 2u || (unsigned long long)nb * bw >= (1ull << 32)) return 0u;
    return 0xFFFFFFFFu / bw + 1u;
}
BH_DEV uint32_t walk_row(uint32_t i, uint32_t bw, uint32_t magic) {
    if (magic) return __umulhi(i, magic);
    if (bw < 2u) return i;
    uint32_t row = (uint32_t)(((float)i + 0.5f) / (float)bw);
    if (row * bw > i) --row;
    else if ((row + 1u) * bw <= i) ++row;
    return row;
}

BH_DEV uint32_t wave_inclusive_scan_u32(uint32_t v, int lane) {
#pragma unroll
    for (int off = 1; off < 64; off <<= 1) {
        const uint32_t t = __shfl_up(v, off);
        if (lane >= off) v += t;
    }
    return v;
}

struct KeepAllTiles { static constexpr bool EAGER = false; BH_DEV bool operator()(const WalkLds&, uint32_t, uint32_t, uint32_t) const { return true; } };
struct KeepLiveTiles {
    static constexpr bool EAGER = false;
    const uint32_t* done_bits;
    uint32_t tile_bw;
    BH_DEV bool operator()(const WalkLds&, uint32_t, uint32_t tx, uint32_t ty) const {
        const uint32_t t = tx + ty * tile_bw;
        return ((done_bits[t >> 5] >> (t & 31u)) & 1u) == 0u;
    }
};
struct KeepNearOfCut {
    const uint32_t* zcut;
    uint32_t tile_bw;
    static constexpr bool EAGER = true;
    BH_DEV uint32_t fetch(uint32_t tx, uint32_t ty) const { return zcut[tx + ty * tile_bw]; }
    BH_DEV bool decide(const WalkLds& w, uint32_t r, uint32_t cut) const { return zcut_near(w.zkey[r], cut); }
    BH_DEV bool operator()(const WalkLds& w, uint32_t r, uint32_t tx, uint32_t ty) const { return decide(w, r, fetch(tx, ty)); }
};

struct NoPrefetch { BH_DEV uint32_t operator()(uint32_t, uint32_t) const { return 0u; } };
template <class OnHit, class Keep = KeepAllTiles, class Pre = NoPrefetch>
BH_DEV uint32_t flat_tile_walk(WalkLds& w, int lane, uint32_t nb, float mx, float my, Sym2 conic, float pt, TileBbox bb,
                               OnHit on_hit, Keep keep = Keep{}, uint32_t zkey = 0u, Pre pre = Pre{}) {
    const uint32_t incl = wave_inclusive_scan_u32(nb, lane);
    const uint32_t start = incl - nb;
    const bool nz = nb > 0u;
    const unsigned long long nzmask = __ballot(nz);
    const unsigned long long below = (1ull << lane) - 1ull;
    const uint32_t rank = (uint32_t)__popcll(nzmask & below);
    const uint32_t bb_w = bb.max_x - bb.min_x;
    if (nz) {
        w.count[rank] = 0;
        w.near[rank] = 0;
        w.zkey[rank] = zkey;
        w.mx[rank] = mx; w.my[rank] = my;
        w.c00[rank] = conic.c00; w.c01[rank] = conic.c01; w.c11[rank] = conic.c11;
        w.pt[rank] = pt;
        w.magic[rank] = walk_magic(bb_w, nb);
        w.box[rank] = bb.min_x | (bb.min_y << 16);
        w.boxw[rank] = bb_w;
        w.start[rank] = start;
        w.lane_of[rank] = (uint32_t)lane;
    }
    __builtin_amdgcn_fence(__ATOMIC_SEQ_CST, "wavefront");
    uint8_t* flags = w.flags;
    const uint32_t tot = __shfl(incl, 63);
    const unsigned long long le = below | (1ull << lane);
    uint32_t before = 0;
    for (uint32_t base = 0; base < tot; base += 64) {
        flags[lane] = 0;
        const uint32_t rel = start - base;
        if (nz && rel < 64u) flags[rel] = 1;
        asm volatile("" ::: "memory");
        const unsigned long long marks = __ballot(flags[lane] != 0);
        asm volatile("" ::: "memory");
        const uint32_t c = base + (uint32_t)lane;
        if (c < tot) {
            const uint32_t r = before + (uint32_t)__popcll(marks & le) - 1u;
            const uint32_t i = c - w.start[r];
            const uint32_t box = w.box[r];
            const uint32_t bw = w.boxw[r];
            const uint32_t row = walk_row(i, bw, w.magic[r]);
            const uint32_t tx = (box & 0xFFFFu) + (i - __umul24(row, bw));
            const uint32_t ty = (box >> 16) + row;
            const uint32_t fetched = pre(tx, ty);
            if (keep(w, r, tx, ty) && will_primitive_contribute(tx, ty, w.mx[r], w.my[r], Sym2{w.c00[r], w.c01[r], w.c11[r]}, w.pt[r])) on_hit(r, tx, ty, fetched);
        }
        before += (uint32_t)__popcll(marks);
    }
    __builtin_amdgcn_fence(__ATOMIC_SEQ_CST, "wavefront");
    return rank;
}

template <class Keep = KeepAllTiles>
BH_DEV uint32_t flat_tile_walk_emit(WalkLds& w, int lane, uint32_t nb, float mx, float my, Sym2 conic, float pt, TileBbox bb,
                                    uint32_t wave_base, uint32_t wave_total, uint32_t tile_bw, uint32_t cg0, uint32_t* __restrict__ tile_ids,
                                    uint32_t* __restrict__ isect_gids, Keep keep = Keep{}, uint32_t zkey = 0u) {
    const uint32_t incl = wave_inclusive_scan_u32(nb, lane);
    const uint32_t start = incl - nb;
    const bool nz = nb > 0u;
    const unsigned long long nzmask = __ballot(nz);
    const unsigned long long below = (1ull << lane) - 1ull;
    const uint32_t rank = (uint32_t)__popcll(nzmask & below);
    const uint32_t bb_w = bb.max_x - bb.min_x;
    if (nz) {
        w.zkey[rank] = zkey;
        w.mx[rank] = mx; w.my[rank] = my;
        w.c00[rank] = conic.c00; w.c01[rank] = conic.c01; w.c11[rank] = conic.c11;
        w.pt[rank] = pt;
        w.magic[rank] = walk_magic(bb_w, nb);
        w.box[rank] = bb.min_x | (bb.min_y << 16);
        w.boxw[rank] = bb_w;
        w.start[rank] = start;
        w.lane_of[rank] = (uint32_t)lane;
    }
    __builtin_amdgcn_fence(__ATOMIC_SEQ_CST, "wavefront");
    uint8_t* flags = w.flags;
    const uint32_t tot = __shfl(incl, 63);
    const unsigned long long le = below | (1ull << lane);
    uint32_t before = 0;
    uint32_t emitted = 0;
    for (uint32_t base = 0; base < tot; base += 64) {
        flags[lane] = 0;
        const uint32_t rel = start - base;
        if (nz && rel < 64u) flags[rel] = 1;
        asm volatile("" ::: "memory");
        const unsigned long long marks = __ballot(flags[lane] != 0);
        asm volatile("" ::: "memory");
        const uint32_t c = base + (uint32_t)lane;
        bool hit = false;
        uint32_t tile = 0, owner = 0;
        if (c < tot) {
            const uint32_t r = before + (uint32_t)__popcll(marks & le) - 1u;
            const uint32_t i = c - w.start[r];
            const uint32_t box = w.box[r];
            const uint32_t bw = w.boxw[r];
            const uint32_t row = walk_row(i, bw, w.magic[r]);
            const uint32_t tx = (box & 0xFFFFu) + (i - __umul24(row, bw));
            const uint32_t ty = (box >> 16) + row;
            if constexpr (Keep::EAGER) {
                const uint32_t cut = keep.fetch(tx, ty);
                uint32_t contributes = will_primitive_contribute(tx, ty, w.mx[r], w.my[r], Sym2{w.c00[r], w.c01[r], w.c11[r]}, w.pt[r]) ? 1u : 0u;
                asm volatile("" : "+v"(contributes));
                hit = contributes != 0u && keep.decide(w, r, cut);
            } else {
                hit = keep(w, r, tx, ty) && will_primitive_contribute(tx, ty, w.mx[r], w.my[r], Sym2{w.c00[r], w.c01[r], w.c11[r]}, w.pt[r]);
            }
            tile = tx + ty * tile_bw;
            owner = cg0 + w.lane_of[r];
        }
        const unsigned long long hits = __ballot(hit);
        if (hit) {
            const uint32_t local = emitted + (uint32_t)__popcll(hits & below);
            if (local < wave_total) {
                tile_ids[wave_base + local] = tile;
                isect_gids[wave_base + local] = owner;
            }
        }
        emitted += (uint32_t)__popcll(hits);
        before += (uint32_t)__popcll(marks);
    }
    for (uint32_t k = emitted + (uint32_t)lane; k < wave_total; k += 64u) {
        tile_ids[wave_base + k] = 0xFFFFFFFFu;
        isect_gids[wave_base + k] = 0u;
    }
    return emitted;
}

template <bool MIP, bool PINHOLE, int DEG>
__global__ __launch_bounds__(PROJ_WG) void project_forward_kernel(
    ViewUniforms u, uint32_t n, const float* __restrict__ transforms, const float* __restrict__ coeffs,
    const float* __restrict__ raw_opacities, uint32_t* __restrict__ depth_keys, uint32_t* __restrict__ isect_counts,
    float* __restrict__ max_radius, float* __restrict__ projected_by_gid, unsigned long long* __restrict__ counters, ForwardPrep prep,
    uint32_t* __restrict__ zcut, uint32_t* __restrict__ near_counts) {
    __shared__ WalkLds s_walk[PROJ_WAVES];
    __shared__ uint32_t s_vis[PROJ_WAVES];
    __shared__ uint32_t s_hit[PROJ_WAVES];
    __shared__ uint32_t s_near[PROJ_WAVES];
    __shared__ uint32_t s_listed[PROJ_WAVES];
    __shared__ uint32_t s_kmax[PROJ_WAVES];
    __shared__ uint32_t s_nmax[PROJ_WAVES];
    __shared__ uint32_t s_bins[ORDER_BINS];
    static_assert(DEAL_SPL_WORDS <= ORDER_BINS, "the splitters are staged in the bins' words");
    uint32_t* const s_spl = s_bins;
    const uint32_t gid = blockIdx.x * PROJ_WG + threadIdx.x;
    if (prep.order_out && blockIdx.x < 8u) {
        const uint32_t per = band_slots(prep.order_tiles);
        __shared__ uint32_t s_band_work, s_band_cnt, s_band_tail, s_band_max;
        for (uint32_t i = threadIdx.x; i < ORDER_BINS; i += PROJ_WG) s_bins[i] = 0u;
        if (threadIdx.x == 0) s_band_work = s_band_cnt = s_band_tail = s_band_max = 0u;
        __syncthreads();
        uint32_t my_work = 0u, my_cnt = 0u, my_max = 0u;
        for (uint32_t i = threadIdx.x; i < per; i += PROJ_WG) {
            const uint32_t lt = band_tile(blockIdx.x, i, per, prep.band_mode);
            if (lt >= prep.order_tiles) continue;
            const uint32_t wk = prep.order_work[prep.order_tile_begin + lt];
            atomicAdd(&s_bins[ORDER_BINS - 1u - (wk < ORDER_BINS ? wk : ORDER_BINS - 1u)], 1u);
            my_work += wk < ORDER_BINS ? wk : ORDER_BINS - 1u;
            my_max = max(my_max, wk < ORDER_BINS ? wk : ORDER_BINS - 1u);
            my_cnt++;
        }
        if (prep.split_out && my_work) atomicAdd(&s_band_work, my_work);
        if (my_cnt) atomicAdd(&s_band_cnt, my_cnt);
        if (prep.split_out && my_max) atomicMax(&s_band_max, my_max);
        __syncthreads();
        const uint32_t cnt = s_band_cnt;
        {
            __shared__ uint32_t s_part[PROJ_WG];
            const uint32_t b0 = threadIdx.x * (ORDER_BINS / PROJ_WG);
            uint32_t loc[ORDER_BINS / PROJ_WG], sum = 0;
#pragma unroll
            for (uint32_t k = 0; k < ORDER_BINS / PROJ_WG; ++k) { loc[k] = sum; sum += s_bins[b0 + k]; }
            s_part[threadIdx.x] = sum;
            __syncthreads();
            if (threadIdx.x == 0) {
                uint32_t run = 0;
                for (uint32_t k = 0; k < (uint32_t)PROJ_WG; ++k) { const uint32_t t = s_part[k]; s_part[k] = run; run += t; }
            }
            __syncthreads();
#pragma unroll
            for (uint32_t k = 0; k < ORDER_BINS / PROJ_WG; ++k) s_bins[b0 + k] = s_part[threadIdx.x] + loc[k];
        }
        __syncthreads();
        if (prep.split_out) {
            if (threadIdx.x == 0) {
                const float mean = cnt ? (float)s_band_work / (float)cnt : 0.0f;
                const float thr_f = fmaxf(fmaxf((float)prep.split_min, prep.split_factor * mean), prep.split_of_max * (float)s_band_max);
                uint32_t h = 0u;
                if (prep.order_mode == 1u && thr_f < (float)(ORDER_BINS - 1u)) {
                    const uint32_t thr = (uint32_t)ceilf(thr_f);
                    h = s_bins[ORDER_BINS - thr];
                }
                prep.split_out[blockIdx.x] = h < SPLIT_MAX ? h : SPLIT_MAX;
            }
            uint32_t* scr = prep.split_out + 8u + blockIdx.x * (SPLIT_MAX * 4u);
            for (uint32_t i = threadIdx.x; i < SPLIT_MAX * 4u; i += PROJ_WG) scr[i] = 0u;
        }
        __syncthreads();
        for (uint32_t i = threadIdx.x; i < per; i += PROJ_WG) {
            const uint32_t lt = band_tile(blockIdx.x, i, per, prep.band_mode);
            if (lt < prep.order_tiles) {
                const uint32_t wk = prep.order_work[prep.order_tile_begin + lt];
                const uint32_t rank = atomicAdd(&s_bins[ORDER_BINS - 1u - (wk < ORDER_BINS ? wk : ORDER_BINS - 1u)], 1u);
                prep.order_out[blockIdx.x * per + rank] = lt;
            } else {
                prep.order_out[blockIdx.x * per + cnt + atomicAdd(&s_band_tail, 1u)] = 0xFFFFFFFFu;
            }
        }
        __syncthreads();
    }
    if (prep.deal.ctr) {
        deal_stage(prep.deal, s_spl);
        __syncthreads();
    }
    if (gid < prep.visible_words) prep.visible[gid] = 0u;
    if (gid < prep.tile_words) prep.tile_table[gid] = 0u;
    if (gid < prep.slice_words) prep.slice_table[gid] = 0u;
    if (gid < COUNTER_SET_U64 && prep.next_counters) prep.next_counters[gid] = 0ull;
    if (gid < DEAL_SET_U64 && prep.deal_next) prep.deal_next[gid] = 0ull;
    for (size_t i = gid; i < prep.span_f4; i += (size_t)gridDim.x * PROJ_WG) prep.span[i] = make_float4(0.0f, 0.0f, 0.0f, 0.0f);
    const int lane = threadIdx.x & 63, wave = threadIdx.x >> 6;
    uint32_t key = 0xFFFFFFFFu;
    float radius = 0.0f;
    bool visible = false;
    float mx = 0.0f, my = 0.0f, pt = 0.0f, opac = 0.0f;
    Sym2 conic = Sym2{0.0f, 0.0f, 0.0f};
    TileBbox bb = TileBbox{0, 0, 0, 0};
    Vec3A mean = v3(0.0f, 0.0f, 0.0f);
    const uint32_t gsafe = gid < n ? gid : (n ? n - 1u : 0u);
    float tr[10];
    {
        const float* trp = transforms + (size_t)gsafe * 10;
#pragma unroll
        for (int k = 0; k < 10; ++k) tr[k] = trp[k];
    }
    float raw_opac = raw_opacities[gsafe];
    constexpr int C_ALL = (DEG + 1) * (DEG + 1);
    float sh_dc[3];
#pragma unroll
    for (int k = 0; k < 3; ++k) sh_dc[k] = coeffs[(size_t)gsafe * C_ALL * 3 + k];
    asm volatile("" : "+v"(tr[0]), "+v"(tr[1]), "+v"(tr[2]), "+v"(tr[3]), "+v"(tr[4]), "+v"(tr[5]), "+v"(tr[6]), "+v"(tr[7]), "+v"(tr[8]), "+v"(tr[9]),
                      "+v"(raw_opac), "+v"(sh_dc[0]), "+v"(sh_dc[1]), "+v"(sh_dc[2]));
    if (gid < n) {
        do {
            mean = v3(tr[0], tr[1], tr[2]);
            const Vec3A mean_c = world_to_cam(mean, u);
            if (!(finite3(mean_c) && mean_c.z <= 1.0e10f)) break;
            if (!in_front_of_camera<PINHOLE>(mean_c, u)) break;
            const Vec3A scl = v3(bh_expf(tr[7]), bh_expf(tr[8]), bh_expf(tr[9]));
            if (!finite3(scl)) break;
            const Quat qu = Quat{tr[3], tr[4], tr[5], tr[6]};
            const float qn = qdot(qu, qu);
            if (!(qn >= 1.0e-6f && is_finite_f32(qn))) break;
            if (!is_finite_f32(raw_opac)) break;
            const Quat q = qnormalize(qu);
            const Sym2 raw_cov = calc_cov2d<PINHOLE>(scl, q, mean_c, u);
            float filter_comp;
            const Sym2 cov = compensate_cov2d<MIP>(raw_cov, filter_comp);
            opac = sigmoid(raw_opac) * filter_comp;
            if (!sym2_finite(cov)) break;
            project_point<PINHOLE>(mean_c, u, mx, my);
            if (!(opac >= 1.0f / 255.0f)) break;
            pt = bh_logf(opac * 255.0f);
            conic = sym2_inverse(cov);
            float ex, ey;
            compute_bbox_extent(conic, pt, ex, ey);
            if (!(ex >= 0.0f && ey >= 0.0f)) break;
            const float wf = (float)u.img_w, hf = (float)u.img_h;
            const bool on_screen = mx + ex > 0.0f && mx - ex < wf && my + ey > 0.0f && my - ey < hf;
            if (!on_screen) break;
            bb = get_tile_bbox(mx, my, ex, ey, u.tile_bw, u.tile_y0, u.tile_y1);
            const bool whole = u.tile_y0 == 0u && u.tile_y1 == u.tile_bh;
            if (!whole && (bb.max_y <= bb.min_y || bb.max_x <= bb.min_x)) break;
            radius = __builtin_fmaxf(ex / wf, ey / hf);
            key = f2u(mean_c.z);
            visible = true;
        } while (false);
    }
    const uint32_t nb = visible ? (bb.max_y - bb.min_y) * (bb.max_x - bb.min_x) : 0u;
    WalkLds& w = s_walk[wave];
    const uint32_t tile_bw = u.tile_bw;
    struct CutOfTile {
        const uint32_t* zcut;
        uint32_t tile_bw;
        BH_DEV uint32_t operator()(uint32_t tx, uint32_t ty) const { return zcut ? zcut[tx + ty * tile_bw] : 0u; }
    };
    const uint32_t wrank = flat_tile_walk(w, lane, nb, mx, my, conic, pt, bb, [&](uint32_t r, uint32_t tx, uint32_t ty, uint32_t cut) {
        atomicAdd(&w.count[r], 1u);
        if (zcut) {
            if (zcut_near(w.zkey[r], cut)) atomicAdd(&w.near[r], 1u);
            else if ((cut & 1u) == 0u) zcut[tx + ty * tile_bw] = cut | 1u;
        }
    }, KeepAllTiles{}, key, CutOfTile{zcut, tile_bw});
    const uint32_t tiles_hit = nb ? w.count[wrank] : 0u;
    const uint32_t near_hit = (nb && zcut) ? w.near[wrank] : 0u;
    const bool listed = visible && (!zcut || near_hit > 0u || prep.list_all_visible);
    constexpr bool DEAL_EARLY = DEG <= 2;
    DealSlot deal_place = DealSlot{0u, 0u};
    if (DEAL_EARLY && prep.deal.ctr && listed) deal_place = deal_take(prep.deal, s_spl, key, zcut ? near_hit : tiles_hit);
    if (listed) {
        const Vec3A v = normalize(sub(mean, camera_pos(u)));
        constexpr int C = (DEG + 1) * (DEG + 1);
        const Vec3A raw = sh_coeffs_to_color_dc<DEG>(coeffs + (size_t)gid * C * 3, v, sh_dc);
        const float cr = raw.x + 0.5f, cgc = raw.y + 0.5f, cb = raw.z + 0.5f;
        float* o = projected_by_gid + (size_t)gid * 9;
        o[0] = mx;
        o[1] = my;
        o[2] = conic.c00;
        o[3] = conic.c01;
        o[4] = conic.c11;
        o[5] = opac;
        o[6] = clampf(is_finite_f32(cr) ? cr : 0.0f, -100.0f, 100.0f);
        o[7] = clampf(is_finite_f32(cgc) ? cgc : 0.0f, -100.0f, 100.0f);
        o[8] = clampf(is_finite_f32(cb) ? cb : 0.0f, -100.0f, 100.0f);
    }
    if (gid < n) {
        depth_keys[gid] = listed ? key : 0xFFFFFFFFu;
        isect_counts[gid] = tiles_hit;
        max_radius[gid] = radius;
        if (zcut) near_counts[gid] = near_hit;
    }
    const unsigned long long ball = __ballot(visible);
    const unsigned long long lball = __ballot(listed);
    uint32_t wave_hits = tiles_hit;
#pragma unroll
    for (int off = 32; off > 0; off >>= 1) wave_hits += __shfl_down(wave_hits, off);
    uint32_t wave_near = 0;
    if (zcut) {
        wave_near = near_hit;
#pragma unroll
        for (int off = 32; off > 0; off >>= 1) wave_near += __shfl_down(wave_near, off);
    }
    uint32_t kmax = listed ? key : 0u, nmax = listed ? ~key : 0u;
#pragma unroll
    for (int off = 32; off > 0; off >>= 1) {
        kmax = max(kmax, (uint32_t)__shfl_xor((int)kmax, off));
        nmax = max(nmax, (uint32_t)__shfl_xor((int)nmax, off));
    }
    if (lane == 0) {
        s_vis[wave] = (uint32_t)__popcll(ball);
        s_hit[wave] = wave_hits;
        s_near[wave] = wave_near;
        s_listed[wave] = (uint32_t)__popcll(lball);
        s_kmax[wave] = kmax;
        s_nmax[wave] = nmax;
    }
    __syncthreads();
    if (!DEAL_EARLY && prep.deal.ctr && listed) deal_place = deal_take(prep.deal, s_spl, key, zcut ? near_hit : tiles_hit);
    if (prep.deal.ctr && listed) deal_put(prep.deal, deal_place, key, gid);
    if (threadIdx.x == 0) {
        uint32_t v = 0, h = 0, nh = 0, ls = 0, km = 0, nm = 0;
#pragma unroll
        for (int k = 0; k < PROJ_WAVES; ++k) { v += s_vis[k]; h += s_hit[k]; nh += s_near[k]; ls += s_listed[k]; km = max(km, s_kmax[k]); nm = max(nm, s_nmax[k]); }
        const uint32_t sl = blockIdx.x & (COUNTER_SLOTS - 1u);
        unsigned long long* slot = counters + COUNTER_K1_U64 * sl;
        if (v) atomicAdd(&slot[0], (unsigned long long)v);
        if (h) atomicAdd(&slot[1], (unsigned long long)h);
        if (nh) atomicAdd(&slot[2], (unsigned long long)nh);
        if (ls && zcut) atomicAdd(&slot[3], (unsigned long long)ls);
        if (ls) {
            uint32_t* mm = reinterpret_cast<uint32_t*>(counters) + COUNTER_MINMAX_WORD + 2u * sl;
            atomicMax(&mm[0], km);
            atomicMax(&mm[1], nm);
        }
    }
}

template <bool MIP, bool PINHOLE>
static int launch_pf_deg(bh_ctx* ctx, const ViewUniforms& u, uint32_t n, uint32_t deg, const float* t, const float* sh, const float* ro,
                         uint32_t* keys, uint32_t* counts, float* radius, float* proj, unsigned long long* c64, const ForwardPrep& prep,
                         uint32_t* zcut, uint32_t* near_counts) {
    const dim3 grid((n + PROJ_WG - 1) / PROJ_WG), block(PROJ_WG);
    switch (deg) {
        case 0: hipLaunchKernelGGL((project_forward_kernel<MIP, PINHOLE, 0>), grid, block, 0, ctx->stream, u, n, t, sh, ro, keys, counts, radius, proj, c64, prep, zcut, near_counts); break;
        case 1: hipLaunchKernelGGL((project_forward_kernel<MIP, PINHOLE, 1>), grid, block, 0, ctx->stream, u, n, t, sh, ro, keys, counts, radius, proj, c64, prep, zcut, near_counts); break;
        case 2: hipLaunchKernelGGL((project_forward_kernel<MIP, PINHOLE, 2>), grid, block, 0, ctx->stream, u, n, t, sh, ro, keys, counts, radius, proj, c64, prep, zcut, near_counts); break;
        case 3: hipLaunchKernelGGL((project_forward_kernel<MIP, PINHOLE, 3>), grid, block, 0, ctx->stream, u, n, t, sh, ro, keys, counts, radius, proj, c64, prep, zcut, near_counts); break;
        case 4: hipLaunchKernelGGL((project_forward_kernel<MIP, PINHOLE, 4>), grid, block, 0, ctx->stream, u, n, t, sh, ro, keys, counts, radius, proj, c64, prep, zcut, near_counts); break;
        default: return set_error(ctx, BH_ERR_INVALID_ARG, "sh_degree must be 0..4");
    }
    BH_LAUNCH_CHECK(ctx, "project_forward_kernel");
    return 0;
}

int launch_project_forward(bh_ctx* ctx, const ViewUniforms& u, uint32_t n, bool mip, uint32_t sh_degree, const float* transforms,
                           const float* sh, const float* raw_opac, uint32_t* depth_keys, uint32_t* isect_counts, float* max_radius,
                           float* projected_by_gid, uint32_t* counters, const ForwardPrep& want, uint32_t* zcut, uint32_t* near_counts) {
    if (zcut && !near_counts) return set_error(ctx, BH_ERR_INVALID_ARG, "project_forward: a depth-cut table needs the near-count output");
    ForwardPrep prep = want;
    const size_t covered = (size_t)((n + PROJ_WG - 1) / PROJ_WG) * PROJ_WG;
    if (prep.visible && prep.visible_words > covered) {
        BH_HIP(ctx, hipMemsetAsync(prep.visible, 0, (size_t)prep.visible_words * 4, ctx->stream));
        prep.visible_words = 0;
    }
    if (prep.next_counters && COUNTER_SET_U64 > covered) {
        BH_HIP(ctx, hipMemsetAsync(prep.next_counters, 0, COUNTER_SET_BYTES, ctx->stream));
        prep.next_counters = nullptr;
    }
    if (prep.deal_next && DEAL_SET_U64 > covered) {
        BH_HIP(ctx, hipMemsetAsync(prep.deal_next, 0, (size_t)DEAL_SET_U64 * 8, ctx->stream));
        prep.deal_next = nullptr;
    }
    if (prep.tile_table && prep.tile_words > covered) {
        BH_HIP(ctx, hipMemsetAsync(prep.tile_table, 0, (size_t)prep.tile_words * 4, ctx->stream));
        prep.tile_words = 0;
    }
    if (prep.slice_table && prep.slice_words > covered) {
        BH_HIP(ctx, hipMemsetAsync(prep.slice_table, 0, (size_t)prep.slice_words * 4, ctx->stream));
        prep.slice_words = 0;
    }
    if (n == 0) {
        if (prep.next_counters) BH_HIP(ctx, hipMemsetAsync(prep.next_counters, 0, COUNTER_SET_BYTES, ctx->stream));
        if (prep.span && prep.span_f4) BH_HIP(ctx, hipMemsetAsync(prep.span, 0, (size_t)prep.span_f4 * 16, ctx->stream));
        return 0;
    }
    auto* c64 = reinterpret_cast<unsigned long long*>(counters);
    const bool pinhole = u.model == CAM_PINHOLE;
    if (mip && pinhole) return launch_pf_deg<true, true>(ctx, u, n, sh_degree, transforms, sh, raw_opac, depth_keys, isect_counts, max_radius, projected_by_gid, c64, prep, zcut, near_counts);
    if (pinhole) return launch_pf_deg<false, true>(ctx, u, n, sh_degree, transforms, sh, raw_opac, depth_keys, isect_counts, max_radius, projected_by_gid, c64, prep, zcut, near_counts);
    if (mip) return launch_pf_deg<true, false>(ctx, u, n, sh_degree, transforms, sh, raw_opac, depth_keys, isect_counts, max_radius, projected_by_gid, c64, prep, zcut, near_counts);
    return launch_pf_deg<false, false>(ctx, u, n, sh_degree, transforms, sh, raw_opac, depth_keys, isect_counts, max_radius, projected_by_gid, c64, prep, zcut, near_counts);
}

__global__ __launch_bounds__(PROJ_WG) void project_visible_kernel(uint32_t nv, const float* __restrict__ projected_by_gid,
                                                                 const uint32_t* __restrict__ global_from_compact_gid,
                                                                 float* __restrict__ projected) {
    const uint32_t e = blockIdx.x * PROJ_WG + threadIdx.x;
    if (e >= nv * 9u) return;
    const uint32_t cg = e / 9u, j = e - cg * 9u;
    projected[e] = projected_by_gid[(size_t)global_from_compact_gid[cg] * 9 + j];
}

int launch_project_visible(bh_ctx* ctx, uint32_t nv, const float* projected_by_gid, const uint32_t* gid, float* projected) {
    if (nv == 0) return 0;
    const uint64_t total = (uint64_t)nv * 9u;
    if (total > 0xFFFFFFFFull) return set_error(ctx, BH_ERR_UNSUPPORTED, "more than 2^32/9 visible splats");
    hipLaunchKernelGGL(project_visible_kernel, dim3((unsigned)((total + PROJ_WG - 1) / PROJ_WG)), dim3(PROJ_WG), 0, ctx->stream, nv,
                       projected_by_gid, gid, projected);
    BH_LAUNCH_CHECK(ctx, "project_visible_kernel");
    return 0;
}
// ... 119 lines not shown
    return (0xFFFFFFFFu >> (31u - (b1 - b0))) << b0;
}

__global__ __launch_bounds__(PROJ_WG) void slice_count_kernel(uint32_t nv, uint32_t tile_bw, uint32_t tile_bh, uint32_t tile_y0, uint32_t tile_y1,
                                                             const float* __restrict__ projected_by_gid,
                                                             const uint32_t* __restrict__ global_from_compact_gid,
                                                             const uint32_t* __restrict__ cum_tiles_hit, uint32_t budget,
                                                             const uint32_t* __restrict__ done_bits, const uint32_t* __restrict__ gate,
                                                             uint32_t* __restrict__ counts, uint32_t* __restrict__ block_totals,
                                                             uint32_t* __restrict__ group_totals, const uint32_t* __restrict__ live_bands) {
    __shared__ WalkLds s_walk[PROJ_WAVES];
    __shared__ uint32_t s_tot[PROJ_WAVES];
    if (*gate == 0u) return;
    const uint32_t live_cols = live_bands[0], live_rows = live_bands[1];
    const uint32_t cg = blockIdx.x * PROJ_WG + threadIdx.x;
    const int lane = threadIdx.x & 63, wave = threadIdx.x >> 6;
    float xy_x = 0.0f, xy_y = 0.0f, pt = 0.0f;
    Sym2 conic = Sym2{0.0f, 0.0f, 0.0f};
    TileBbox bb = TileBbox{0, 0, 0, 0};
    uint32_t nb = 0;
    if (cg < nv && cum_tiles_hit[cg] > budget) {
        const float* src = projected_by_gid + (size_t)global_from_compact_gid[cg] * 9;
        xy_x = src[0]; xy_y = src[1];
        conic = Sym2{src[2], src[3], src[4]};
        pt = bh_logf(src[5] * 255.0f);
        float ex, ey;
        compute_bbox_extent(conic, pt, ex, ey);
        bb = get_tile_bbox(xy_x, xy_y, ex, ey, tile_bw, tile_y0, tile_y1);
        nb = (bb.max_y - bb.min_y) * (bb.max_x - bb.min_x);
        if (nb) {
            if ((band_mask(bb.min_x, bb.max_x, tile_bw) & live_cols) == 0u || (band_mask(bb.min_y, bb.max_y, tile_bh) & live_rows) == 0u) nb = 0u;
        }
    }
    WalkLds& w = s_walk[wave];
    uint32_t hits = 0;
    if (__ballot(nb > 0u) != 0ull) {
        const uint32_t wrank = flat_tile_walk(w, lane, nb, xy_x, xy_y, conic, pt, bb, [&](uint32_t r, uint32_t, uint32_t, uint32_t) { atomicAdd(&w.count[r], 1u); },
                                              KeepLiveTiles{done_bits, tile_bw});
        hits = nb ? w.count[wrank] : 0u;
    }
    if (cg < nv) counts[cg] = hits;
    uint32_t wsum = hits;
#pragma unroll
    for (int off = 32; off > 0; off >>= 1) wsum += __shfl_down(wsum, off);
    if (lane == 0) s_tot[wave] = wsum;
    __syncthreads();
    if (threadIdx.x == 0) {
        uint32_t t = 0;
#pragma unroll
        for (int w = 0; w < PROJ_WAVES; ++w) t += s_tot[w];
        block_totals[blockIdx.x] = t;
        if (t) atomicAdd(group_totals + blockIdx.x / FAR_GROUP_BLOCKS, t);
    }
}

int launch_map_gaussians(bh_ctx* ctx, uint32_t nv, const ViewUniforms& u, const float* projected_by_gid, const uint32_t* gid,
                         float* projected, const uint32_t* cum_tiles_hit, uint32_t* tile_ids, uint32_t* isect_gids,
                         float4* zero_span, uint32_t zero_f4, uint32_t budget, uint32_t* slice_info, const uint32_t* zcut,
                         const uint32_t* depth_keys_sorted, const uint32_t* nv_dev, uint32_t pair_cap) {
    if (nv == 0) return 0;
    if (zcut && (!slice_info || !depth_keys_sorted)) return set_error(ctx, BH_ERR_INVALID_ARG, "map_gaussians: a depth-cut table needs the slice words and the sorted keys");
    const dim3 grid((nv + PROJ_WG - 1) / PROJ_WG), block(PROJ_WG);
    const uint32_t* nul = nullptr;
    if (slice_info) {
#define BH_K5_SPW 16
        constexpr int SPW = BH_K5_SPW;
        const dim3 grid16((nv + PROJ_WAVES * SPW - 1) / (PROJ_WAVES * SPW));
        hipLaunchKernelGGL((map_gaussians_kernel<false, SPW>), grid16, block, 0, ctx->stream, nv, u.tile_bw, u.tile_bh, u.tile_y0, u.tile_y1, projected_by_gid, gid,
                           projected, cum_tiles_hit, tile_ids, isect_gids, zero_span, zero_f4, budget, slice_info, nul, nul, nul, nul, nul, zcut, depth_keys_sorted, nv_dev, pair_cap);
    } else if (ctx->knob_k5_exact_spw != 64u) {
        const uint32_t spw = ctx->knob_k5_exact_spw == 16u ? 16u : 32u;
        const dim3 gridn((nv + PROJ_WAVES * spw - 1) / (PROJ_WAVES * spw));
        if (spw == 16u)
            hipLaunchKernelGGL((map_gaussians_kernel<false, 16>), gridn, block, 0, ctx->stream, nv, u.tile_bw, u.tile_bh, u.tile_y0, u.tile_y1, projected_by_gid, gid,
                               projected, cum_tiles_hit, tile_ids, isect_gids, zero_span, zero_f4, budget, slice_info, nul, nul, nul, nul, nul, nul, nul, nv_dev, pair_cap);
        else
            hipLaunchKernelGGL((map_gaussians_kernel<false, 32>), gridn, block, 0, ctx->stream, nv, u.tile_bw, u.tile_bh, u.tile_y0, u.tile_y1, projected_by_gid, gid,
                               projected, cum_tiles_hit, tile_ids, isect_gids, zero_span, zero_f4, budget, slice_info, nul, nul, nul, nul, nul, nul, nul, nv_dev, pair_cap);
    } else {
        hipLaunchKernelGGL((map_gaussians_kernel<false, 64>), grid, block, 0, ctx->stream, nv, u.tile_bw, u.tile_bh, u.tile_y0, u.tile_y1, projected_by_gid, gid,
                           projected, cum_tiles_hit, tile_ids, isect_gids, zero_span, zero_f4, budget, slice_info, nul, nul, nul, nul, nul, nul, nul, nv_dev, pair_cap);
    }
    BH_LAUNCH_CHECK(ctx, "map_gaussians_kernel");
    return 0;
}

int launch_map_gaussians_far(bh_ctx* ctx, uint32_t nv, const ViewUniforms& u, const float* projected_by_gid, const uint32_t* gid,
                             float* projected, const uint32_t* cum_tiles_hit, uint32_t budget, const uint32_t* done_bits, const uint32_t* gate,
                             uint32_t* counts, uint32_t* block_totals, uint32_t* group_totals, uint32_t* slice_info, uint32_t* tile_ids,
                             uint32_t* isect_gids) {
    if (nv == 0) return 0;
    const dim3 grid((nv + PROJ_WG - 1) / PROJ_WG), block(PROJ_WG);
    hipLaunchKernelGGL(slice_count_kernel, grid, block, 0, ctx->stream, nv, u.tile_bw, u.tile_bh, u.tile_y0, u.tile_y1, projected_by_gid, gid, cum_tiles_hit,
                       budget, done_bits, gate, counts, block_totals, group_totals, (const uint32_t*)(slice_info + 4));
    BH_LAUNCH_CHECK(ctx, "slice_count_kernel");
    hipLaunchKernelGGL((map_gaussians_kernel<true, 64>), grid, block, 0, ctx->stream, nv, u.tile_bw, u.tile_bh, u.tile_y0, u.tile_y1, projected_by_gid, gid,
                       projected, cum_tiles_hit, tile_ids, isect_gids, (float4*)nullptr, 0u, budget, slice_info, (const uint32_t*)counts,
                       (const uint32_t*)block_totals, (const uint32_t*)group_totals, done_bits, gate, (const uint32_t*)nullptr, (const uint32_t*)nullptr, (const uint32_t*)nullptr, 0xFFFFFFFFu);
    BH_LAUNCH_CHECK(ctx, "map_gaussians_kernel<far>");
    return 0;
}

BH_DEV Quat apply_normalize_vjp(Quat q, Quat g) {
    const float lsq = qdot(q, q);
    const float l = __builtin_sqrtf(lsq);
    const float inv = 1.0f / (l * lsq);
    const float qw = q.w, qx = q.x, qy = q.y, qz = q.z;
    const float gw = g.w, gx = g.x, gy = g.y, gz = g.z;
    const float cc0 = -qw * qx, cc1 = -qx * qy, cc2 = -qy * qw;
    const float cs0 = -qw * qz, cs1 = -qx * qz, cs2 = -qy * qz;
    const float sw = qw * qw, sx = qx * qx, sy = qy * qy, sz = qz * qz;
    return Quat{((lsq - sw) * gw + cc0 * gx + cc2 * gy + cs0 * gz) * inv,
                (cc0 * gw + (lsq - sx) * gx + cc1 * gy + cs1 * gz) * inv,
                (cc2 * gw + cc1 * gx + (lsq - sy) * gy + cs2 * gz) * inv,
                (cs0 * gw + cs1 * gx + cs2 * gy + (lsq - sz) * gz) * inv};
}
BH_DEV Quat quat_to_mat_vjp(Quat q, const Mat3& v) {
    const float qw = q.w, qx = q.x, qy = q.y, qz = q.z;
    const float w_grad = qx * (v.c1z - v.c2y) + qy * (v.c2x - v.c0z) + qz * (v.c0y - v.c1x);
    const float x_grad = -2.0f * qx * (v.c1y + v.c2z) + qy * (v.c0y + v.c1x) + qz * (v.c0z + v.c2x) + qw * (v.c1z - v.c2y);
    const float y_grad = qx * (v.c0y + v.c1x) - 2.0f * qy * (v.c0x + v.c2z) + qz * (v.c1z + v.c2y) + qw * (v.c2x - v.c0z);
    const float z_grad = qx * (v.c0z + v.c2x) + qy * (v.c1z + v.c2y) - 2.0f * qz * (v.c0x + v.c1y) + qw * (v.c0y - v.c1x);
    return Quat{2.0f * w_grad, 2.0f * x_grad, 2.0f * y_grad, 2.0f * z_grad};
}
BH_DEV Vec3A projection_vjp_pinhole(const Mat2x3& jac, Vec3A mean_c, Sym3 cov_c, const ViewUniforms& u, Sym2 v_cov2d, Vec2 v_mean2d) {
    const float fx = u.fx, fy = u.fy;
    const float mx = mean_c.x, my = mean_c.y, mz = mean_c.z;
    const float inv_z = 1.0f / mz;
    const float mx_rz_raw = mx * inv_z, my_rz_raw = my * inv_z;
    const float mx_rz = clampf(mx_rz_raw, u.lim_neg_x, u.lim_pos_x);
    const float my_rz = clampf(my_rz_raw, u.lim_neg_y, u.lim_pos_y);
    const bool in_x = mx_rz_raw <= u.lim_pos_x && mx_rz_raw >= u.lim_neg_x;
    const bool in_y = my_rz_raw <= u.lim_pos_y && my_rz_raw >= u.lim_neg_y;
    const float inv_z2 = inv_z * inv_z;
    const float inv_z3 = inv_z2 * inv_z;
    float v_mx = fx * inv_z * v_mean2d.x;
    float v_my = fy * inv_z * v_mean2d.y;
    float v_mz = -(fx * mx * v_mean2d.x + fy * my * v_mean2d.y) * inv_z2;
    const Mat2x3 tmp = sym2_mul_mat2x3(v_cov2d, jac);
    const float vj00 = 2.0f * dot(row0(tmp), s3row0(cov_c));
    const float vj11 = 2.0f * dot(row1(tmp), s3row1(cov_c));
    const float vj20 = 2.0f * dot(row0(tmp), s3row2(cov_c));
    const float vj21 = 2.0f * dot(row1(tmp), s3row2(cov_c));
    const float tx = mz * mx_rz;
    const float ty = mz * my_rz;
    if (in_x) v_mx += -fx * inv_z2 * vj20; else v_mz += -fx * inv_z3 * vj20 * tx;
    if (in_y) v_my += -fy * inv_z2 * vj21; else v_mz += -fy * inv_z3 * vj21 * ty;
    v_mz += -fx * inv_z2 * vj00 - fy * inv_z2 * vj11 + 2.0f * fx * tx * inv_z3 * vj20 + 2.0f * fy * ty * inv_z3 * vj21;
    return Vec3A{v_mx, v_my, v_mz};
}

template <bool MIP, int DEG, bool PINHOLE>
__global__ __launch_bounds__(PROJ_WG) void project_backward_kernel(
    ViewUniforms u, uint32_t nv, const float* __restrict__ transforms, const float* __restrict__ sh_coeffs,
    const float* __restrict__ raw_opac, const uint32_t* __restrict__ global_from_compact_gid,
    float* __restrict__ v_combined, float* __restrict__ v_transforms, float* __restrict__ v_coeffs,
    float* __restrict__ v_raw_opac, float* __restrict__ v_refine_weight, const bool mark_written, const float* __restrict__ projected) {
    const uint32_t cg = blockIdx.x * PROJ_WG + threadIdx.x;
    if (cg >= nv) return;
    uint32_t gid = global_from_compact_gid[cg];
    float* rg = v_combined + (size_t)cg * 10;
    float g[10];
    bool any = false;
#pragma unroll
    for (int k = 0; k < 10; ++k) g[k] = rg[k];
    asm volatile("" : "+v"(gid));
// ... 221 lines not shown
```

Before: 1388.

## Stage near tile pairs in K1 and copy them in K5 on cut-list frames

```diff
diff --git a/brush_amd/_ffi.py b/brush_amd/_ffi.py
--- a/brush_amd/_ffi.py
+++ b/brush_amd/_ffi.py
@@ -478,6 +478,9 @@
                                                        C.c_uint32, C.c_uint32, C.POINTER(C.c_uint64), C.POINTER(C.c_int)]),
                      "bh_debug_dsort_deal_counts": (C.c_int, [C.c_void_p, C.POINTER(C.c_uint32)]),
                      "bh_debug_set_deal_capacity": (C.c_int, [C.c_void_p, C.c_uint32]),
+                     "bh_debug_set_stage_capacity": (C.c_int, [C.c_void_p, C.c_uint32]),
+                     "bh_debug_k1_lists_counts": (C.c_int, [C.c_void_p, C.POINTER(C.c_uint32)]),
+                     "bh_debug_last_view_cuts": (C.c_int, [C.c_void_p, C.c_void_p, C.c_uint32]),
                      "bh_debug_image_loss_window": (C.c_int, [C.c_void_p, C.c_void_p, C.c_void_p, C.c_uint32, C.c_uint32, C.POINTER(BhLossConfig), C.c_float, C.c_uint32,
                                                               C.c_uint32, C.c_void_p, C.c_void_p])}
 
diff --git a/brush_amd/csrc/api.hip b/brush_amd/csrc/api.hip
--- a/brush_amd/csrc/api.hip
+++ b/brush_amd/csrc/api.hip
@@ -272,6 +272,7 @@
     if (ctx->host_counters) (void)hipHostFree(ctx->host_counters);
     if (ctx->dsort_spl) (void)hipFree(ctx->dsort_spl);
     if (ctx->deal_ctr) (void)hipFree(ctx->deal_ctr);
+    if (ctx->stage_cursors) (void)hipFree(ctx->stage_cursors);
     if (ctx->sort_groups) (void)hipFree(ctx->sort_groups);
     if (ctx->readback_ev) (void)hipEventDestroy(ctx->readback_ev);
     if (ctx->gate_ev) (void)hipEventDestroy(ctx->gate_ev);
@@ -384,6 +385,8 @@
      [](bh_ctx* c, const char* v) { return parse_flag(v, &c->knob_dsort_splitters); }},
     {"dsort_deal", "0|1: K1 deals the listed splats straight into the depth sort's buckets when the view's splitter table holds quantiles (default 1) or the histogram and split launches always run",
      [](bh_ctx* c, const char* v) { return parse_flag(v, &c->knob_dsort_deal); }},
+    {"k1_lists", "0|1: on cut-list frames K1 stages the near pairs its walk finds and K5 copies them (default 1) or K5 walks the listed splats' candidates again",
+     [](bh_ctx* c, const char* v) { return parse_flag(v, &c->knob_k1_lists); }},
     {"tile_sort", "auto|bucket|lsd: the forward's tile sort (auto: bucket sort unless the view's pairs are concentrated in few tiles)",
      [](bh_ctx* c, const char* v) { const std::string w(v); if (w == "auto") { c->knob_tile_sort = 0; return true; } if (w == "bucket") { c->knob_tile_sort = 1; return true; } if (w == "lsd") { c->knob_tile_sort = 2; return true; } return false; }},
     {"spec_k5", "0|1: queue the list builder before the host has read the frame's counts (default 1; 0: behind the count readback)",
@@ -686,6 +689,7 @@
     uint32_t* cum_early = nullptr;
     bool k5_queued = false;
     uint32_t spec_pair_cap = 0;
+    StageArgs staged;
     float* spec_projected = nullptr;
     float4* spec_vc = nullptr;
     uint32_t *spec_tile_ids = nullptr, *spec_isect_gids = nullptr;
@@ -736,6 +740,29 @@
             }
             BH_TRY(depth_deal_prepare(ctx, n, spl, sums_on_device && spl_written && *spl_written && depth_deal_table_usable(*spl_listed), &prep));
             dealt = prep.deal;
+            if (ctx->knob_k1_lists && sums_on_device) {
+                if (ctx->stage_cursors == nullptr) {
+                    constexpr size_t set_bytes = (size_t)STAGE_CURSORS * STAGE_CURSOR_STRIDE * sizeof(uint32_t);
+                    if (hipMalloc((void**)&ctx->stage_cursors, 2 * set_bytes) != hipSuccess) { (void)hipGetLastError(); ctx->stage_cursors = nullptr; return BH_ERR_OOM; }
+                    BH_HIP(ctx, hipMemsetAsync(ctx->stage_cursors, 0, 2 * set_bytes, ctx->stream));
+                    ctx->stage_phase = 0u;
+                }
+                prep.stage_measure = true;
+                prep.stage_next = ctx->stage_cursors + (size_t)STAGE_CURSORS * STAGE_CURSOR_STRIDE * ((ctx->stage_phase & 1u) ^ 1u);
+                const uint32_t cap_blocks = ctx->stage_cap_override ? (ctx->stage_cap_override + STAGE_BLOCK - 1u) / STAGE_BLOCK : ctx->stage_cap_blocks;
+                const bool room_known = ctx->stage_cap_override || (cap_blocks > 0u && ctx->stage_need_blocks <= cap_blocks);
+                if (cut_active && room_known && f.num_tiles <= STAGE_MAX_TILES) {
+                    const uint32_t region_blocks = (cap_blocks + STAGE_CURSORS - 1u) / STAGE_CURSORS;
+                    staged.buf = (uint16_t*)ensure(ctx, SLOT_STAGE_TILES, (size_t)region_blocks * STAGE_CURSORS * STAGE_BLOCK * sizeof(uint16_t));
+                    staged.start = (uint32_t*)ensure(ctx, SLOT_STAGE_START, npad * 4);
+                    if (!staged.buf || !staged.start) return BH_ERR_OOM;
+                    staged.cursor = ctx->stage_cursors + (size_t)STAGE_CURSORS * STAGE_CURSOR_STRIDE * (ctx->stage_phase & 1u);
+                    staged.region_blocks = region_blocks;
+                    prep.stage = staged;
+                    ctx->stage_frames++;
+                }
+                ctx->stage_phase ^= 1u;
+            }
             BH_TRY(launch_project_forward(ctx, f.u, n, mip, sh_degree, transforms, sh_coeffs, raw_opacities, depth_keys, isect_counts, max_radius,
                                           f.proj_by_gid, counters, prep, cut_active ? vtab : nullptr, near_counts));
             ctx->counter_phase ^= 1u;
@@ -770,6 +797,10 @@
                 spec_isect_gids = (uint32_t*)ctx->slots[SLOT_ISECT_GIDS].ptr;
                 spec_pair_cap = (uint32_t)std::min<size_t>(cap_pairs, 0xFFFFFFFEull);
                 ProfScope ps(ctx, "MapGaussiansToIntersect");
+                if (staged.buf)
+                    BH_TRY(launch_copy_staged_pairs(ctx, n, f.proj_by_gid, f.gfc, spec_projected, cum_early, spec_tile_ids, spec_isect_gids, spec_vc,
+                                                    spec_vc ? (uint32_t)(((size_t)n * 10 + 3) / 4) : 0u, slice_tab, dev_sums + 3, spec_pair_cap, staged, dev_sums + COUNTER_K1_U64));
+                else
                 BH_TRY(launch_map_gaussians(ctx, n, f.u, f.proj_by_gid, f.gfc, spec_projected, cum_early, spec_tile_ids, spec_isect_gids, spec_vc,
                                             spec_vc ? (uint32_t)(((size_t)n * 10 + 3) / 4) : 0u, 0xFFFFFFFFu, cut_active ? slice_tab : nullptr,
                                             cut_active ? vtab : nullptr, cut_active ? depths_sorted : nullptr, dev_sums + (cut_active ? 3 : 0), spec_pair_cap));
@@ -789,6 +820,21 @@
         } else {
             for (uint32_t k = 0; k < COUNTER_SLOTS; ++k)
                 for (uint32_t c = 0; c < COUNTER_K1_U64; ++c) hc[c] += hslots[COUNTER_K1_U64 * k + c];
+        }
+        const uint64_t stage_need = hc[0] >> 32, stage_full = hc[2] >> 32;
+        hc[0] &= 0xFFFFFFFFull;
+        hc[2] &= 0xFFFFFFFFull;
+        if (stage_need > ctx->stage_need_blocks) ctx->stage_need_blocks = (uint32_t)stage_need;
+        if (ctx->stage_need_blocks > 0u && (uint64_t)ctx->stage_need_blocks + ctx->stage_need_blocks / 16u > ctx->stage_cap_blocks) {
+            const uint64_t want = (uint64_t)ctx->stage_need_blocks + ctx->stage_need_blocks / 2u + 64u;
+            const uint32_t room = (uint32_t)std::min<uint64_t>(want, STAGE_MAX_BLOCKS);
+            if (room > ctx->stage_cap_blocks) ctx->stage_cap_blocks = room;
+        }
+        if (staged.buf && stage_full != 0u) {
+            ctx->stage_fallbacks++;
+            if (!ctx->stage_cap_override) ctx->stage_cap_blocks = (uint32_t)std::min<uint64_t>((uint64_t)ctx->stage_cap_blocks + ctx->stage_cap_blocks / 4u, STAGE_MAX_BLOCKS);
+            staged = StageArgs{};
+            k5_queued = false;
         }
         if (hc[1] > 0xFFFFFFFFull) return set_error(ctx, BH_ERR_UNSUPPORTED, "more than 2^32-1 tile intersections");
         nv_true = (uint32_t)hc[0];
@@ -852,6 +898,8 @@
         f.rs.split = tile_split;
 #ifdef BH_TEST_HOOKS
         ctx->last_split = tile_split;
+        ctx->last_view_table = vtab;
+        ctx->last_view_tiles = f.num_tiles;
 #endif
     }
     const uint32_t win_tiles = f.u.tile_bw * (f.u.tile_y1 - f.u.tile_y0);
@@ -884,6 +932,10 @@
                     ctx->clears.k5_cleared_accum(vc != nullptr);
                 } else {
                     ctx->clears.k5_cleared_accum(vc != nullptr);
+                    if (staged.buf && zcut_lists)
+                        BH_TRY(launch_copy_staged_pairs(ctx, f.nv, f.proj_by_gid, f.gfc, f.projected, f.cum, f.tile_ids, f.isect_gids, vc, vc ? (uint32_t)(((size_t)f.nv * 10 + 3) / 4) : 0u,
+                                                        f.slice_info, nullptr, 0xFFFFFFFFu, staged, nullptr));
+                    else
                     BH_TRY(launch_map_gaussians(ctx, f.nv, f.u, f.proj_by_gid, f.gfc, f.projected, f.cum, f.tile_ids, f.isect_gids, vc, vc ? (uint32_t)(((size_t)f.nv * 10 + 3) / 4) : 0u,
                                                 (sliced && !by_cut) ? f.budget : 0xFFFFFFFFu, (sliced || zcut_lists) ? f.slice_info : nullptr, zcut_lists,
                                                 zcut_lists ? depths_sorted : nullptr));
@@ -1453,6 +1505,24 @@
     ctx->deal_cap_override = cap;
     return 0;
 }
+extern "C" int bh_debug_set_stage_capacity(bh_ctx* ctx, uint32_t entries) {
+    if (!ctx) return BH_ERR_INVALID_ARG;
+    ctx->stage_cap_override = entries;
+    return 0;
+}
+extern "C" int bh_debug_last_view_cuts(bh_ctx* ctx, uint32_t* out, uint32_t tiles) {
+    if (!ctx || !out) return BH_ERR_INVALID_ARG;
+    if (!ctx->last_view_table || tiles != ctx->last_view_tiles) return set_error(ctx, BH_ERR_STATE, "debug_last_view_cuts: the last forward had no view table of that many tiles");
+    BH_HIP(ctx, hipStreamSynchronize(ctx->stream));
+    BH_HIP(ctx, hipMemcpy(out, ctx->last_view_table, (size_t)tiles * 4, hipMemcpyDeviceToHost));
+    return 0;
+}
+extern "C" int bh_debug_k1_lists_counts(bh_ctx* ctx, uint32_t* out) {
+    if (!ctx || !out) return BH_ERR_INVALID_ARG;
+    out[0] = ctx->stage_frames;
+    out[1] = ctx->stage_fallbacks;
+    return 0;
+}
 extern "C" int bh_debug_dsort_deal_counts(bh_ctx* ctx, uint32_t* out) {
     if (!ctx || !out) return BH_ERR_INVALID_ARG;
     out[0] = ctx->deal_frames;
diff --git a/brush_amd/csrc/context.h b/brush_amd/csrc/context.h
--- a/brush_amd/csrc/context.h
+++ b/brush_amd/csrc/context.h
@@ -98,6 +98,8 @@
     SLOT_FEATURE_GRAD,
     SLOT_ENVMAP_FRAME,
     SLOT_DEAL_REGION,
+    SLOT_STAGE_TILES,
+    SLOT_STAGE_START,
     SLOT_SCENE,
     SLOT_SPTSDF,
     SLOT_COUNT
@@ -193,6 +195,17 @@
     unsigned long long* ctr = nullptr;
     uint2* region = nullptr;
     uint32_t cap = 0;
+};
+constexpr uint32_t STAGE_BLOCK = 64;
+constexpr uint32_t STAGE_CURSORS = 128;
+constexpr uint32_t STAGE_CURSOR_STRIDE = 32;
+constexpr uint32_t STAGE_MAX_BLOCKS = 1u << 21;
+constexpr uint32_t STAGE_MAX_TILES = 65536;
+struct StageArgs {
+    uint16_t* buf = nullptr;
+    uint32_t* start = nullptr;
+    uint32_t* cursor = nullptr;
+    uint32_t region_blocks = 0;
 };
 constexpr size_t MAX_VIEW_STATES = 4096;
 constexpr uint64_t DIRECT_ALLREDUCE_MIN_FLOATS = 1u << 16;
@@ -437,6 +450,8 @@
     uint32_t knob_k16_split_min = bh::SPLIT_MIN_WORK;
     uint32_t knob_k16_split_of_max = 45;
     const uint32_t* last_split = nullptr;
+    const uint32_t* last_view_table = nullptr;
+    uint32_t last_view_tiles = 0;
     uint32_t knob_k16_order = 1;
     uint32_t knob_cut_margin_pct = 150;
     bh::FarJob far_job;
@@ -453,6 +468,13 @@
     uint32_t deal_phase = 0;
     uint32_t deal_frames = 0, deal_fallbacks = 0;
     uint32_t deal_cap_override = 0;
+    uint32_t* stage_cursors = nullptr;
+    uint32_t stage_phase = 0;
+    uint32_t stage_cap_blocks = 0;
+    uint32_t stage_need_blocks = 0;
+    uint32_t stage_frames = 0, stage_fallbacks = 0;
+    uint32_t stage_cap_override = 0;
+    bool knob_k1_lists = true;
     bool knob_dsort_deal = true;
     bool knob_dsort_splitters = true;
     bool adam_lds_raised = false;
@@ -613,6 +635,9 @@
     bool list_all_visible = false;
     DealArgs deal;
     unsigned long long* deal_next = nullptr;
+    StageArgs stage;
+    uint32_t* stage_next = nullptr;
+    bool stage_measure = false;
 };
 int launch_project_forward(bh_ctx* ctx, const ViewUniforms& u, uint32_t n, bool mip, uint32_t sh_degree, const float* transforms,
                            const float* sh, const float* raw_opac, uint32_t* depth_keys, uint32_t* isect_counts, float* max_radius,
@@ -623,6 +648,9 @@
                          float* projected, const uint32_t* cum_tiles_hit, uint32_t* tile_ids, uint32_t* isect_gids,
                          float4* zero_span = nullptr, uint32_t zero_f4 = 0, uint32_t budget = 0xFFFFFFFFu, uint32_t* slice_info = nullptr,
                          const uint32_t* zcut = nullptr, const uint32_t* depth_keys_sorted = nullptr, const uint32_t* nv_dev = nullptr, uint32_t pair_cap = 0xFFFFFFFFu);
+int launch_copy_staged_pairs(bh_ctx* ctx, uint32_t nv, const float* projected_by_gid, const uint32_t* gid, float* projected,
+                             const uint32_t* cum_tiles_hit, uint32_t* tile_ids, uint32_t* isect_gids, float4* zero_span, uint32_t zero_f4,
+                             uint32_t* slice_info, const uint32_t* nv_dev, uint32_t pair_cap, const StageArgs& stage, const uint32_t* stage_ovf);
 int launch_map_gaussians_far(bh_ctx* ctx, uint32_t nv, const ViewUniforms& u, const float* projected_by_gid, const uint32_t* gid,
                              float* projected, const uint32_t* cum_tiles_hit, uint32_t budget, const uint32_t* done_bits, const uint32_t* gate,
                              uint32_t* counts, uint32_t* block_totals, uint32_t* group_totals, uint32_t* slice_info, uint32_t* tile_ids, uint32_t* isect_gids);
diff --git a/brush_amd/csrc/depth_sort.hip b/brush_amd/csrc/depth_sort.hip
--- a/brush_amd/csrc/depth_sort.hip
+++ b/brush_amd/csrc/depth_sort.hip
@@ -111,7 +111,11 @@
     if (lane == 0) {
         if (dev_sums) {
 #pragma unroll
-            for (uint32_t c = 0; c < COUNTER_K1_U64; ++c) dev_sums[c] = deal_overflow ? 0u : (tot[c] > 0xFFFFFFFFull ? 0xFFFFFFFFu : (uint32_t)tot[c]);
+            for (uint32_t c = 0; c < COUNTER_K1_U64; ++c) {
+                const unsigned long long t = (c == 0u || c == 2u) ? (tot[c] & 0xFFFFFFFFull) : tot[c];
+                dev_sums[c] = deal_overflow ? 0u : (t > 0xFFFFFFFFull ? 0xFFFFFFFFu : (uint32_t)t);
+            }
+            dev_sums[COUNTER_K1_U64] = (uint32_t)(tot[2] >> 32);
         }
         volatile unsigned long long* h64 = reinterpret_cast<volatile unsigned long long*>(host_sums);
 #pragma unroll
diff --git a/brush_amd/csrc/project.hip b/brush_amd/csrc/project.hip
--- a/brush_amd/csrc/project.hip
+++ b/brush_amd/csrc/project.hip
@@ -45,6 +45,17 @@
     return v;
 }
 
+BH_DEV uint32_t wave_inclusive_scan_u32_fresh(uint32_t v, int lane) {
+    int l = lane;
+    asm volatile("" : "+v"(l));
+#pragma unroll
+    for (int off = 1; off < 64; off <<= 1) {
+        const uint32_t t = (uint32_t)__builtin_amdgcn_ds_bpermute((l >= off ? l - off : l) << 2, (int)v);
+        if (l >= off) v += t;
+    }
+    return v;
+}
+
 struct KeepAllTiles { static constexpr bool EAGER = false; BH_DEV bool operator()(const WalkLds&, uint32_t, uint32_t, uint32_t) const { return true; } };
 struct KeepLiveTiles {
     static constexpr bool EAGER = false;
@@ -65,10 +76,49 @@
 };
 
 struct NoPrefetch { BH_DEV uint32_t operator()(uint32_t, uint32_t) const { return 0u; } };
-template <class OnHit, class Keep = KeepAllTiles, class Pre = NoPrefetch>
+struct NoStage {
+    static constexpr bool ON = false;
+    BH_DEV void begin(uint32_t, int) {}
+    BH_DEV void step(unsigned long long, uint32_t) {}
+};
+struct StageNear {
+    static constexpr bool ON = true;
+    StageArgs to;
+    uint32_t need = 0;
+    uint32_t emitted = 0;
+    uint32_t ticket = 0;
+    BH_DEV void begin(uint32_t tot , int lane) {
+        need = (tot + STAGE_BLOCK - 1u) / STAGE_BLOCK;
+        if (to.buf && need && lane == 0) {
+            uint32_t zero = 0u;
+            asm volatile("" : "+v"(zero));
+            ticket = atomicAdd(to.cursor + (blockIdx.x & (STAGE_CURSORS - 1u)) * STAGE_CURSOR_STRIDE + zero, need);
+        }
+    }
+    BH_DEV uint32_t first_block() const {
+        uint32_t t = ticket;
+        asm volatile("" : "+v"(t));
+        return (uint32_t)__builtin_amdgcn_readfirstlane((int)t);
+    }
+    BH_DEV bool fits(uint32_t blk) const { return blk <= to.region_blocks && need <= to.region_blocks - blk; }
+    BH_DEV uint32_t room(uint32_t blk) const { return ((blockIdx.x & (STAGE_CURSORS - 1u)) * to.region_blocks + blk) * STAGE_BLOCK; }
+    static constexpr uint32_t NOT_NEAR = 0xFFFFFFFFu;
+    BH_DEV void step(unsigned long long below, uint32_t near_tile ) {
+        if (to.buf == nullptr) return;
+        const bool near = near_tile != NOT_NEAR;
+        const unsigned long long nears = __ballot(near);
+        if (nears == 0ull) return;
+        const uint32_t blk = first_block();
+        if (near && fits(blk)) to.buf[(size_t)room(blk) + emitted + (uint32_t)__popcll(nears & below)] = (uint16_t)near_tile;
+        emitted += (uint32_t)__popcll(nears);
+    }
+};
+template <class OnHit, class Keep = KeepAllTiles, class Pre = NoPrefetch, class Stage = NoStage>
 BH_DEV uint32_t flat_tile_walk(WalkLds& w, int lane, uint32_t nb, float mx, float my, Sym2 conic, float pt, TileBbox bb,
-                               OnHit on_hit, Keep keep = Keep{}, uint32_t zkey = 0u, Pre pre = Pre{}) {
+                               OnHit on_hit, Keep keep = Keep{}, uint32_t zkey = 0u, Pre pre = Pre{}, Stage* stage = nullptr) {
     const uint32_t incl = wave_inclusive_scan_u32(nb, lane);
+    const uint32_t tot = __shfl(incl, 63);
+    if constexpr (Stage::ON) stage->begin((uint32_t)__builtin_amdgcn_readlane((int)incl, 63), lane);
     const uint32_t start = incl - nb;
     const bool nz = nb > 0u;
     const unsigned long long nzmask = __ballot(nz);
@@ -90,7 +140,6 @@
     }
     __builtin_amdgcn_fence(__ATOMIC_SEQ_CST, "wavefront");
     uint8_t* flags = w.flags;
-    const uint32_t tot = __shfl(incl, 63);
     const unsigned long long le = below | (1ull << lane);
     uint32_t before = 0;
     for (uint32_t base = 0; base < tot; base += 64) {
@@ -101,6 +150,7 @@
         const unsigned long long marks = __ballot(flags[lane] != 0);
         asm volatile("" ::: "memory");
         const uint32_t c = base + (uint32_t)lane;
+        uint32_t near_tile = 0xFFFFFFFFu;
         if (c < tot) {
             const uint32_t r = before + (uint32_t)__popcll(marks & le) - 1u;
             const uint32_t i = c - w.start[r];
@@ -110,8 +160,12 @@
             const uint32_t tx = (box & 0xFFFFu) + (i - __umul24(row, bw));
             const uint32_t ty = (box >> 16) + row;
             const uint32_t fetched = pre(tx, ty);
-            if (keep(w, r, tx, ty) && will_primitive_contribute(tx, ty, w.mx[r], w.my[r], Sym2{w.c00[r], w.c01[r], w.c11[r]}, w.pt[r])) on_hit(r, tx, ty, fetched);
-        }
+            if (keep(w, r, tx, ty) && will_primitive_contribute(tx, ty, w.mx[r], w.my[r], Sym2{w.c00[r], w.c01[r], w.c11[r]}, w.pt[r])) {
+                if constexpr (Stage::ON) near_tile = on_hit(r, tx, ty, fetched);
+                else on_hit(r, tx, ty, fetched);
+            }
+        }
+        if constexpr (Stage::ON) stage->step(below, near_tile);
         before += (uint32_t)__popcll(marks);
     }
     __builtin_amdgcn_fence(__ATOMIC_SEQ_CST, "wavefront");
@@ -206,6 +260,7 @@
     __shared__ uint32_t s_listed[PROJ_WAVES];
     __shared__ uint32_t s_kmax[PROJ_WAVES];
     __shared__ uint32_t s_nmax[PROJ_WAVES];
+    __shared__ uint32_t s_room[PROJ_WAVES];
     __shared__ uint32_t s_bins[ORDER_BINS];
     static_assert(DEAL_SPL_WORDS <= ORDER_BINS, "the splitters are staged in the bins' words");
     uint32_t* const s_spl = s_bins;
@@ -284,6 +339,7 @@
     if (gid < prep.slice_words) prep.slice_table[gid] = 0u;
     if (gid < COUNTER_SET_U64 && prep.next_counters) prep.next_counters[gid] = 0ull;
     if (gid < DEAL_SET_U64 && prep.deal_next) prep.deal_next[gid] = 0ull;
+    if (gid < STAGE_CURSORS && prep.stage_next) prep.stage_next[gid * STAGE_CURSOR_STRIDE] = 0u;
     for (size_t i = gid; i < prep.span_f4; i += (size_t)gridDim.x * PROJ_WG) prep.span[i] = make_float4(0.0f, 0.0f, 0.0f, 0.0f);
     const int lane = threadIdx.x & 63, wave = threadIdx.x >> 6;
     uint32_t key = 0xFFFFFFFFu;
@@ -351,15 +407,25 @@
         uint32_t tile_bw;
         BH_DEV uint32_t operator()(uint32_t tx, uint32_t ty) const { return zcut ? zcut[tx + ty * tile_bw] : 0u; }
     };
+    StageNear staging;
+    staging.to = prep.stage;
     const uint32_t wrank = flat_tile_walk(w, lane, nb, mx, my, conic, pt, bb, [&](uint32_t r, uint32_t tx, uint32_t ty, uint32_t cut) {
         atomicAdd(&w.count[r], 1u);
         if (zcut) {
-            if (zcut_near(w.zkey[r], cut)) atomicAdd(&w.near[r], 1u);
+            if (zcut_near(w.zkey[r], cut)) { atomicAdd(&w.near[r], 1u); return tx + ty * tile_bw; }
             else if ((cut & 1u) == 0u) zcut[tx + ty * tile_bw] = cut | 1u;
         }
-    }, KeepAllTiles{}, key, CutOfTile{zcut, tile_bw});
+        return StageNear::NOT_NEAR;
+    }, KeepAllTiles{}, key, CutOfTile{zcut, tile_bw}, &staging);
     const uint32_t tiles_hit = nb ? w.count[wrank] : 0u;
     const uint32_t near_hit = (nb && zcut) ? w.near[wrank] : 0u;
+    bool stage_full = false;
+    if (staging.to.buf && staging.emitted) {
+        const uint32_t ahead = wave_inclusive_scan_u32_fresh(near_hit, lane) - near_hit;
+        const uint32_t blk = staging.first_block();
+        if (!staging.fits(blk)) stage_full = true;
+        else if (near_hit) staging.to.start[gid] = staging.room(blk) + ahead;
+    }
     const bool listed = visible && (!zcut || near_hit > 0u || prep.list_all_visible);
     constexpr bool DEAL_EARLY = DEG <= 2;
     DealSlot deal_place = DealSlot{0u, 0u};
@@ -410,19 +476,24 @@
         s_listed[wave] = (uint32_t)__popcll(lball);
         s_kmax[wave] = kmax;
         s_nmax[wave] = nmax;
+        s_room[wave] = (prep.stage_measure ? staging.need : 0u) | (stage_full ? 0x80000000u : 0u);
     }
     __syncthreads();
     if (!DEAL_EARLY && prep.deal.ctr && listed) deal_place = deal_take(prep.deal, s_spl, key, zcut ? near_hit : tiles_hit);
     if (prep.deal.ctr && listed) deal_put(prep.deal, deal_place, key, gid);
     if (threadIdx.x == 0) {
         uint32_t v = 0, h = 0, nh = 0, ls = 0, km = 0, nm = 0;
-#pragma unroll
-        for (int k = 0; k < PROJ_WAVES; ++k) { v += s_vis[k]; h += s_hit[k]; nh += s_near[k]; ls += s_listed[k]; km = max(km, s_kmax[k]); nm = max(nm, s_nmax[k]); }
+        unsigned long long room = 0ull, full = 0ull;
+#pragma unroll
+        for (int k = 0; k < PROJ_WAVES; ++k) {
+            v += s_vis[k]; h += s_hit[k]; nh += s_near[k]; ls += s_listed[k]; km = max(km, s_kmax[k]); nm = max(nm, s_nmax[k]);
+            room += s_room[k] & 0x7FFFFFFFu; full += s_room[k] >> 31;
+        }
         const uint32_t sl = blockIdx.x & (COUNTER_SLOTS - 1u);
         unsigned long long* slot = counters + COUNTER_K1_U64 * sl;
-        if (v) atomicAdd(&slot[0], (unsigned long long)v);
+        if (v) atomicAdd(&slot[0], (unsigned long long)v | (room << 32));
         if (h) atomicAdd(&slot[1], (unsigned long long)h);
-        if (nh) atomicAdd(&slot[2], (unsigned long long)nh);
+        if (nh) atomicAdd(&slot[2], (unsigned long long)nh | (full << 32));
         if (ls && zcut) atomicAdd(&slot[3], (unsigned long long)ls);
         if (ls) {
             uint32_t* mm = reinterpret_cast<uint32_t*>(counters) + COUNTER_MINMAX_WORD + 2u * sl;
@@ -708,6 +779,87 @@
                            projected, cum_tiles_hit, tile_ids, isect_gids, zero_span, zero_f4, budget, slice_info, nul, nul, nul, nul, nul, nul, nul, nv_dev, pair_cap);
     }
     BH_LAUNCH_CHECK(ctx, "map_gaussians_kernel");
+    return 0;
+}
+
+template <int SPW>
+__global__ __launch_bounds__(PROJ_WG) void copy_staged_pairs_kernel(
+    uint32_t nv, const float* __restrict__ projected_by_gid, const uint32_t* __restrict__ global_from_compact_gid, float* __restrict__ projected,
+    const uint32_t* __restrict__ cum_tiles_hit, uint32_t* __restrict__ tile_id_from_isect, uint32_t* __restrict__ compact_gid_from_isect,
+    float4* __restrict__ zero_span, uint32_t zero_f4, uint32_t* __restrict__ slice_info, const uint32_t* __restrict__ nv_dev, uint32_t pair_cap,
+    const uint16_t* __restrict__ stage, const uint32_t* __restrict__ stage_start, uint32_t stage_entries, const uint32_t* __restrict__ stage_ovf) {
+    static_assert(SPW >= 2 && SPW <= 64 && (SPW & (SPW - 1)) == 0, "the owner search halves SPW");
+    __shared__ uint32_t s_end[PROJ_WAVES][SPW];
+    __shared__ uint32_t s_src[PROJ_WAVES][SPW];
+    if (stage_ovf && *stage_ovf != 0u) return;
+    if (nv_dev) {
+        const uint32_t live = *nv_dev;
+        nv = live < nv ? live : nv;
+        const size_t zf = ((size_t)nv * 10 + 3) / 4;
+        zero_f4 = zf < (size_t)zero_f4 ? (uint32_t)zf : zero_f4;
+    }
+    const uint32_t tid_lin = blockIdx.x * PROJ_WG + threadIdx.x;
+    for (size_t i = tid_lin; i < zero_f4; i += (size_t)gridDim.x * PROJ_WG) zero_span[i] = make_float4(0.0f, 0.0f, 0.0f, 0.0f);
+    const int lane = threadIdx.x & 63, wave = threadIdx.x >> 6;
+    const uint32_t cg0 = (blockIdx.x * PROJ_WAVES + (uint32_t)wave) * (uint32_t)SPW;
+    const uint32_t cg = lane < SPW ? cg0 + (uint32_t)lane : 0xFFFFFFFFu;
+    uint32_t base = 0, end = 0, run = 0;
+    bool mine = false;
+    if (cg < nv) {
+        uint32_t cum_end = cum_tiles_hit[cg];
+        uint32_t cum_prev = cum_tiles_hit[cg == 0u ? 0u : cg - 1u];
+        uint32_t my_gid = global_from_compact_gid[cg];
+        asm volatile("" : "+v"(cum_end), "+v"(cum_prev), "+v"(my_gid));
+        if (cg == 0u) cum_prev = 0u;
+        base = cum_prev;
+        end = cum_end;
+        mine = end > base;
+        if (slice_info && cg + 1u == nv) { slice_info[0] = nv; slice_info[1] = cum_end; }
+        if (mine) {
+            run = stage_start[my_gid];
+            const float* src = projected_by_gid + (size_t)my_gid * 9;
+            float p[9];
+#pragma unroll
+            for (int k = 0; k < 9; ++k) p[k] = src[k];
+            float* dst = projected + (size_t)cg * 9;
+#pragma unroll
+            for (int k = 0; k < 9; ++k) dst[k] = p[k];
+        }
+    }
+    const unsigned long long mine_mask = __ballot(mine);
+    if (mine_mask == 0ull) return;
+    const int first_lane = __builtin_ctzll(mine_mask), last_lane = 63 - __builtin_clzll(mine_mask);
+    const uint32_t wave_base = __shfl(base, first_lane);
+    const uint32_t wave_total = __shfl(end, last_lane) - wave_base;
+    if (wave_base > pair_cap || wave_total > pair_cap - wave_base) return;
+    if (lane < SPW) {
+        s_end[wave][lane] = cg < nv ? (end > wave_base ? end - wave_base : 0u) : wave_total;
+        s_src[wave][lane] = run - (base - wave_base);
+    }
+    __builtin_amdgcn_fence(__ATOMIC_SEQ_CST, "wavefront");
+    asm volatile("" ::: "memory");
+    const uint32_t* ends = s_end[wave];
+    for (uint32_t k = (uint32_t)lane; k < wave_total; k += 64u) {
+        uint32_t owner = 0;
+#pragma unroll
+        for (uint32_t step = SPW / 2; step != 0u; step >>= 1) owner += ends[owner + step - 1u] <= k ? step : 0u;
+        const uint32_t e = s_src[wave][owner] + k;
+        tile_id_from_isect[wave_base + k] = e < stage_entries ? (uint32_t)stage[e] : 0xFFFFFFFFu;
+        compact_gid_from_isect[wave_base + k] = e < stage_entries ? cg0 + owner : 0u;
+    }
+}
+
+int launch_copy_staged_pairs(bh_ctx* ctx, uint32_t nv, const float* projected_by_gid, const uint32_t* gid, float* projected,
+                             const uint32_t* cum_tiles_hit, uint32_t* tile_ids, uint32_t* isect_gids, float4* zero_span, uint32_t zero_f4,
+                             uint32_t* slice_info, const uint32_t* nv_dev, uint32_t pair_cap, const StageArgs& stage, const uint32_t* stage_ovf) {
+    if (nv == 0) return 0;
+    if (!slice_info || !stage.buf || !stage.start) return set_error(ctx, BH_ERR_INVALID_ARG, "copy_staged_pairs: the slice words and the staging buffers are needed");
+    constexpr int SPW = BH_K5_SPW;
+    const dim3 grid((nv + PROJ_WAVES * SPW - 1) / (PROJ_WAVES * SPW)), block(PROJ_WG);
+    hipLaunchKernelGGL((copy_staged_pairs_kernel<SPW>), grid, block, 0, ctx->stream, nv, projected_by_gid, gid, projected, cum_tiles_hit, tile_ids, isect_gids,
+                       zero_span, zero_f4, slice_info, nv_dev, pair_cap, (const uint16_t*)stage.buf, (const uint32_t*)stage.start,
+                       stage.region_blocks * STAGE_CURSORS * STAGE_BLOCK, stage_ovf);
+    BH_LAUNCH_CHECK(ctx, "copy_staged_pairs_kernel");
     return 0;
 }
 
```

Result: no change. 1382 (-0.4%).
